# yannikkellerde/TD3

Hardware: AMD Instinct MI355X
Metric: TD3 gradient-steps/sec @ batch 256, HalfCheetah-v4, 1/2/4/8 GPU (higher is better)
Workload: dtype f32; 1 GPU; TD3_featured.train(replay_buffer, 256) on HalfCheetah-v4 shapes (state 17, action 6, actor 500-400-300, critic 2x 500-400-200, LayerNorm, policy_freq 2), replay 1e6 per GPU; global_batch=256, per_gpu_batch=256, replay_per_gpu=1000000, parallelism=single, launch=auto, norm=layer

## Files before the change

include/td3.h:

```cpp
#ifndef TD3_HIP_H
#define TD3_HIP_H

#include <stddef.h>
#include <stdint.h>

#ifdef __cplusplus
extern "C" {
#endif

typedef struct rb_handle rb_handle;
typedef struct td3_handle td3_handle;

typedef struct rb_info_t {
  int state_dim, action_dim;
  int record_floats;
  int64_t max_size, ptr, size;
  void* data;
  int device;
  int n_particles, particle_dim;
} rb_info_t;

int rb_create(int state_dim, int action_dim, int64_t max_size, int device, uint64_t seed,
              rb_handle** out);
int rb_destroy(rb_handle* h);
// ... 54 lines not shown
  double actor_loss;
  int actor_step;
  float* y;
  float* q1;
  float* q2;
  int64_t* idx;
  float* noise;
} td3_step_stats;

size_t td3_config_size(void);
int td3_default_config(td3_config* cfg, size_t cfg_size);
int td3_create(const td3_config* cfg, td3_handle** out);
int td3_destroy(td3_handle* h);

int td3_tensor_count(const td3_handle* h, int which_group );
int td3_tensor_info(const td3_handle* h, int which_group, int index, char* name, int name_len,
                    int64_t* rows, int64_t* cols);
int64_t td3_num_params(const td3_handle* h, int which_group);
int td3_get_params(td3_handle* h, int which, float* out, int64_t n);
int td3_set_params(td3_handle* h, int which, const float* in, int64_t n);
int td3_get_counters(const td3_handle* h, int64_t* total_it, int64_t* critic_step,
                     int64_t* actor_step);
int td3_set_counters(td3_handle* h, int64_t total_it, int64_t critic_step, int64_t actor_step);
int td3_set_adam(td3_handle* h, int group, double lr, double beta1, double beta2, double eps);
int td3_get_adam(const td3_handle* h, int group, double out[4] );

int td3_train_step(td3_handle* h, rb_handle* rb, int batch, void* stream,
                   const int64_t* inject_idx, const float* inject_noise, td3_step_stats* stats);
int td3_train_step_batch(td3_handle* h, const float* state, const float* action,
                         const float* next_state, const float* reward, const float* not_done,
                         int batch, void* stream, const float* inject_noise,
                         td3_step_stats* stats);
int td3_select_action(td3_handle* h, const float* state, float* action_out, int n);
int td3_eval_q(td3_handle* h, const float* state, const float* action, float* q_out, int n);

typedef struct td3_explore {
  float* x;
  float mu, theta, sigma;
  const uint8_t* reset;
  uint64_t seed, step;
  const float* inject_z;
  float* z_out;
} td3_explore;
int td3_select_action_device(td3_handle* h, const float* state, int n, const td3_explore* ex,
                             float* action_out, void* stream);
int td3_eval_q_device(td3_handle* h, const float* state, const float* action, int n, float* q_out, void* stream);

int td3_train_step_batch_particles(td3_handle* h, const float* feat, const float* part, const float* action,
                                   const float* next_feat, const float* next_part, const float* reward,
                                   const float* not_done, int batch, void* stream, const float* inject_noise,
                                   td3_step_stats* stats);
int td3_actor_learn_particles(td3_handle* h, const float* feat, const float* part, int batch, void* stream,
                              double* actor_loss);
int td3_select_action_particles(td3_handle* h, const float* feat, const float* part, float* action_out, int n);
int td3_eval_q_particles(td3_handle* h, const float* feat, const float* part, const float* action, float* q_out,
                         int n);
int td3_select_action_particles_device(td3_handle* h, const float* feat, const float* part, int n,
                                       const td3_explore* ex, float* action_out, void* stream);
int td3_eval_q_particles_device(td3_handle* h, const float* feat, const float* part, const float* action,
                                int n, float* q_out, void* stream);

int td3_comm_unique_id(unsigned char out[128]);
int td3_comm_init(td3_handle* h, const unsigned char id[128], int nranks, int rank);
int td3_dp_gather_optimizer_state(td3_handle* h);
int td3_comm_init_local(td3_handle** hs, int n);
int td3_train_step_local(td3_handle** hs, rb_handle** rbs, int n, int batch, const int64_t* inject_idx,
                         const float* inject_noise, td3_step_stats* stats);

int td3_sync(td3_handle* h);
void* td3_stream(td3_handle* h);
int td3_profile_stages(td3_handle* h, rb_handle* rb, int batch, int actor_phase, float* ms,
                       int max_stages, int* n_stages);
const char* td3_stage_name(td3_handle* h, int i);
const char* td3_stage_kernel(td3_handle* h, int i);
int td3_time_stage(td3_handle* h, int stage, int iters, float* ms_mean);
int td3_probe_kernel(td3_handle* h, rb_handle* rb, int batch, const char* kernel, int steps, float* ms_total,
                     int* launches);
double td3_stage_flops(td3_handle* h, int i);
double td3_stage_bytes(td3_handle* h, int i);
int td3_debug_activation(td3_handle* h, int eval, int layer, float* out, int rows, int cols);
int td3_debug_plan_flags(const td3_handle* h, int* flags);

int td3_debug_act_fail(td3_handle* h, int n);

const char* td3_last_error(void);

#ifdef __cplusplus
}
#endif
#endif
```

td3_amd/_lib.py:

```python
from __future__ import annotations

import atexit
import ctypes as C
import os

_HERE = os.path.dirname(os.path.abspath(__file__))
LIB_PATH = os.path.join(_HERE, "libtd3hip.so")


class rb_info_t(C.Structure):
    _fields_ = [("state_dim", C.c_int), ("action_dim", C.c_int), ("record_floats", C.c_int),
                ("max_size", C.c_int64), ("ptr", C.c_int64), ("size", C.c_int64),
                ("data", C.c_void_p), ("device", C.c_int),
                ("n_particles", C.c_int), ("particle_dim", C.c_int)]


class td3_config(C.Structure):
    _fields_ = [("struct_size", C.c_int), ("state_dim", C.c_int), ("action_dim", C.c_int),
                ("actor_hidden", C.c_int * 3), ("critic_hidden", C.c_int * 3),
                ("norm", C.c_int), ("max_action", C.c_float),
                ("discount", C.c_double), ("tau", C.c_double), ("policy_noise", C.c_double),
                ("noise_clip", C.c_double), ("policy_freq", C.c_int),
                ("lr", C.c_double), ("beta1", C.c_double), ("beta2", C.c_double),
                ("eps", C.c_double), ("seed", C.c_uint64), ("device", C.c_int),
# ... 1 lines not shown
                ("particle_dim", C.c_int), ("cdq", C.c_int)]


class td3_step_stats(C.Structure):
    _fields_ = [("critic_loss", C.c_double), ("actor_loss", C.c_double), ("actor_step", C.c_int),
                ("y", C.c_void_p), ("q1", C.c_void_p), ("q2", C.c_void_p), ("idx", C.c_void_p),
                ("noise", C.c_void_p)]


class td3_explore(C.Structure):
    _fields_ = [("x", C.c_void_p), ("mu", C.c_float), ("theta", C.c_float), ("sigma", C.c_float),
                ("reset", C.c_void_p), ("seed", C.c_uint64), ("step", C.c_uint64),
                ("inject_z", C.c_void_p), ("z_out", C.c_void_p)]


_P = C.c_void_p
_F = C.POINTER(C.c_float)
_D = C.POINTER(C.c_double)
_I64 = C.POINTER(C.c_int64)

SIGNATURES = {
    "rb_create": (C.c_int, [C.c_int, C.c_int, C.c_int64, C.c_int, C.c_uint64, C.POINTER(_P)]),
    "rb_destroy": (C.c_int, [_P]),
    "rb_info": (C.c_int, [_P, C.POINTER(rb_info_t)]),
    "rb_stream": (_P, [_P]),
    "rb_add": (C.c_int, [_P, _D, _D, _D, _D, _D, C.c_int64, _P]),
    "rb_add_records": (C.c_int, [_P, _F, C.c_int64, _P]),
    "rb_add_device": (C.c_int, [_P, _P, _P, _P, _P, _P, C.c_int64, _P]),
    "rb_add_particles_device": (C.c_int, [_P, _P, _P, _P, _P, _P, _P, _P, C.c_int64, _P]),
    "rb_fill_synthetic": (C.c_int, [_P, C.c_int64, C.c_float, C.c_uint64, _P]),
    "rb_sample": (C.c_int, [_P, C.c_int, _P, _P, _P, _P, _P, _P, _P, _P]),
    "rb_read_records": (C.c_int, [_P, C.c_int64, C.c_int64, _F]),
    "rb_write_records": (C.c_int, [_P, C.c_int64, C.c_int64, _F, C.c_int64, C.c_int64]),
    "rb_sync": (C.c_int, [_P]),
    "rb_create_particles": (C.c_int, [C.c_int, C.c_int, C.c_int, C.c_int, C.c_int64, C.c_int, C.c_uint64,
                                      C.POINTER(_P)]),
    "rb_add_particles": (C.c_int, [_P, _D, _D, _D, _D, _D, _D, _D, C.c_int64, _P]),
    "rb_sample_particles": (C.c_int, [_P, C.c_int, _P, _P, _P, _P, _P, _P, _P, _P, _P, _P]),
    "td3_config_size": (C.c_size_t, []),
    "td3_default_config": (C.c_int, [C.POINTER(td3_config), C.c_size_t]),
    "td3_create": (C.c_int, [C.POINTER(td3_config), C.POINTER(_P)]),
    "td3_destroy": (C.c_int, [_P]),
    "td3_tensor_count": (C.c_int, [_P, C.c_int]),
    "td3_tensor_info": (C.c_int, [_P, C.c_int, C.c_int, C.c_char_p, C.c_int, _I64, _I64]),
    "td3_num_params": (C.c_int64, [_P, C.c_int]),
    "td3_get_params": (C.c_int, [_P, C.c_int, _F, C.c_int64]),
    "td3_set_params": (C.c_int, [_P, C.c_int, _F, C.c_int64]),
    "td3_get_counters": (C.c_int, [_P, _I64, _I64, _I64]),
    "td3_set_counters": (C.c_int, [_P, C.c_int64, C.c_int64, C.c_int64]),
    "td3_set_adam": (C.c_int, [_P, C.c_int, C.c_double, C.c_double, C.c_double, C.c_double]),
    "td3_get_adam": (C.c_int, [_P, C.c_int, _D]),
    "td3_train_step": (C.c_int, [_P, _P, C.c_int, _P, _I64, _F, C.POINTER(td3_step_stats)]),
    "td3_train_step_batch": (C.c_int, [_P, _P, _P, _P, _P, _P, C.c_int, _P, _F,
                                       C.POINTER(td3_step_stats)]),
    "td3_select_action": (C.c_int, [_P, _F, _F, C.c_int]),
    "td3_eval_q": (C.c_int, [_P, _F, _F, _F, C.c_int]),
    "td3_select_action_device": (C.c_int, [_P, _P, C.c_int, C.POINTER(td3_explore), _P, _P]),
    "td3_eval_q_device": (C.c_int, [_P, _P, _P, C.c_int, _P, _P]),
    "td3_select_action_particles_device": (C.c_int, [_P, _P, _P, C.c_int, C.POINTER(td3_explore), _P, _P]),
    "td3_eval_q_particles_device": (C.c_int, [_P, _P, _P, _P, C.c_int, _P, _P]),
    "td3_train_step_batch_particles": (C.c_int, [_P, _P, _P, _P, _P, _P, _P, _P, C.c_int, _P, _F,
                                                 C.POINTER(td3_step_stats)]),
    "td3_actor_learn_particles": (C.c_int, [_P, _P, _P, C.c_int, _P, _D]),
    "td3_select_action_particles": (C.c_int, [_P, _F, _F, _F, C.c_int]),
    "td3_eval_q_particles": (C.c_int, [_P, _F, _F, _F, _F, C.c_int]),
    "td3_comm_unique_id": (C.c_int, [C.POINTER(C.c_ubyte)]),
    "td3_comm_init": (C.c_int, [_P, C.POINTER(C.c_ubyte), C.c_int, C.c_int]),
    "td3_comm_init_local": (C.c_int, [C.POINTER(_P), C.c_int]),
    "td3_dp_gather_optimizer_state": (C.c_int, [_P]),
    "td3_train_step_local": (C.c_int, [C.POINTER(_P), C.POINTER(_P), C.c_int, C.c_int, _I64, _F,
                                       C.POINTER(td3_step_stats)]),
    "td3_sync": (C.c_int, [_P]),
    "td3_stream": (_P, [_P]),
    "td3_profile_stages": (C.c_int, [_P, _P, C.c_int, C.c_int, _F, C.c_int, C.POINTER(C.c_int)]),
    "td3_stage_name": (C.c_char_p, [_P, C.c_int]),
    "td3_stage_kernel": (C.c_char_p, [_P, C.c_int]),
    "td3_time_stage": (C.c_int, [_P, C.c_int, C.c_int, _F]),
    "td3_probe_kernel": (C.c_int, [_P, _P, C.c_int, C.c_char_p, C.c_int, _F, C.POINTER(C.c_int)]),
    "td3_stage_flops": (C.c_double, [_P, C.c_int]),
    "td3_stage_bytes": (C.c_double, [_P, C.c_int]),
    "td3_debug_activation": (C.c_int, [_P, C.c_int, C.c_int, _P, C.c_int, C.c_int]),
    "td3_debug_plan_flags": (C.c_int, [_P, _P]),
    "td3_debug_act_fail": (C.c_int, [_P, C.c_int]),
    "td3_last_error": (C.c_char_p, []),
}

TD3_ACTOR, TD3_ACTOR_TARGET, TD3_CRITIC, TD3_CRITIC_TARGET = 0, 1, 2, 3
TD3_ACTOR_ADAM_M, TD3_ACTOR_ADAM_V, TD3_CRITIC_ADAM_M, TD3_CRITIC_ADAM_V = 4, 5, 6, 7
TD3_ACTOR_GRAD, TD3_CRITIC_GRAD = 8, 9

_lib = None
_shutting_down = False


def _mark_shutdown():
    global _shutting_down
    _shutting_down = True


atexit.register(_mark_shutdown)


def alive() -> bool:
    return _lib is not None and not _shutting_down


def load(path: str = LIB_PATH):
    global _lib
    if _lib is not None:
        return _lib
    import torch
    path = os.environ.get("TD3_LIB", path)
    if not os.path.exists(path):
        raise ImportError(
            f"libtd3hip.so not found at {path}: build it with `python -m td3_amd.build` "
            "(hipcc --offload-arch=gfx950). There is no CPU fallback.")
    lib = C.CDLL(path, mode=C.RTLD_GLOBAL)
    for name, (res, args) in SIGNATURES.items():
        fn = getattr(lib, name)
        fn.restype = res
        fn.argtypes = args
    _lib = lib
    return lib


class TD3Error(RuntimeError):
    pass


def check(rc: int, what: str = ""):
    if rc != 0:
        msg = _lib.td3_last_error().decode(errors="replace") if _lib is not None else ""
        raise TD3Error(f"{what} failed ({rc}): {msg}")


def default_config():
    lib = load()
    if C.sizeof(td3_config) != lib.td3_config_size():
        raise TD3Error(f"td3_config binding is {C.sizeof(td3_config)} bytes, libtd3hip's "
                       f"{lib.td3_config_size()}: td3_amd/_lib.py is out of date with include/td3.h")
    cfg = td3_config()
    check(lib.td3_default_config(C.byref(cfg), C.sizeof(cfg)), "td3_default_config")
    return cfg


def fptr(a):
    return a.ctypes.data_as(_F)


def i64ptr(a):
    return a.ctypes.data_as(_I64)


def dptr(a):
    return a.ctypes.data_as(_D)
```

td3_amd/csrc/common.h:

```cpp
#pragma once
#include <hip/hip_runtime.h>
#include <stdint.h>
#include <stddef.h>

#define TD3_EV_FLAGS (hipEventDisableTiming | hipEventReleaseToDevice)

namespace td3 {
void set_error(const char* fmt, ...);
}

#define TD3_HIP(expr)                                                              \
  do {                                                                             \
    hipError_t _e = (expr);                                                        \
    if (_e != hipSuccess) {                                                        \
      td3::set_error("%s:%d %s -> %s", __FILE__, __LINE__, #expr,                  \
                     hipGetErrorString(_e));                                       \
      return -2;                                                                   \
    }                                                                              \
  } while (0)

#define TD3_ARG(cond, msg)                                                         \
  do {                                                                             \
    if (!(cond)) {                                                                 \
      td3::set_error("argument error: %s (%s)", msg, #cond);                        \
// ... 1 lines not shown
    }                                                                              \
  } while (0)

#define TD3_RC(expr)          \
  do {                        \
    int _rc = (expr);         \
    if (_rc) return _rc;      \
  } while (0)

namespace td3 {

constexpr int kWave = 64;
constexpr int kTile = 32;

__host__ __device__ inline int pad32(int x) { return (x + 31) & ~31; }
__host__ __device__ inline int pad4(int x) { return (x + 3) & ~3; }

__host__ __device__ inline int lds_stride(int kp) { return kp + ((4 - kp) % 64 + 64) % 64; }

struct u32x4 { uint32_t x, y, z, w; };

__device__ __forceinline__ u32x4 philox4x32_10(u32x4 ctr, uint32_t k0, uint32_t k1) {
  const uint32_t M0 = 0xD2511F53u, M1 = 0xCD9E8D57u;
  const uint32_t W0 = 0x9E3779B9u, W1 = 0xBB67AE85u;
#pragma unroll
  for (int i = 0; i < 10; ++i) {
    uint32_t hi0 = __umulhi(M0, ctr.x), lo0 = M0 * ctr.x;
    uint32_t hi1 = __umulhi(M1, ctr.z), lo1 = M1 * ctr.z;
    ctr = u32x4{hi1 ^ ctr.y ^ k0, lo1, hi0 ^ ctr.w ^ k1, lo0};
    k0 += W0;
    k1 += W1;
  }
  return ctr;
}

enum : uint32_t { kStreamIndex = 1u, kStreamNoise = 2u, kStreamFill = 3u, kStreamExplore = 4u };

__device__ __forceinline__ uint64_t philox_index(uint64_t seed, uint64_t step, uint32_t row,
                                                 uint64_t n) {
  u32x4 c{row, kStreamIndex, (uint32_t)step, (uint32_t)(step >> 32)};
  u32x4 r = philox4x32_10(c, (uint32_t)seed, (uint32_t)(seed >> 32));
  uint64_t bits = ((uint64_t)r.x << 32) | r.y;
  return __umul64hi(bits, n);
}

__device__ __forceinline__ float u01_open(uint32_t x) {
  return ((float)(x >> 8) + 1.0f) * (1.0f / 16777216.0f);
}

__device__ __forceinline__ void philox_normal4(uint64_t seed, uint64_t step, uint32_t stream,
                                               uint32_t idx, float out[4]) {
  u32x4 c{idx, stream, (uint32_t)step, (uint32_t)(step >> 32)};
  u32x4 r = philox4x32_10(c, (uint32_t)seed, (uint32_t)(seed >> 32));
  float u1 = u01_open(r.x), u2 = u01_open(r.y), u3 = u01_open(r.z), u4 = u01_open(r.w);
  constexpr float kM2Ln2 = -2.0f * 0.693147180559945f;
  const float rad1 = __builtin_amdgcn_sqrtf(kM2Ln2 * __builtin_amdgcn_logf(u1));
  const float rad2 = __builtin_amdgcn_sqrtf(kM2Ln2 * __builtin_amdgcn_logf(u3));
  const float s1 = __builtin_amdgcn_sinf(u2), c1 = __builtin_amdgcn_cosf(u2);
  const float s2 = __builtin_amdgcn_sinf(u4), c2 = __builtin_amdgcn_cosf(u4);
  out[0] = rad1 * c1;
  out[1] = rad1 * s1;
  out[2] = rad2 * c2;
  out[3] = rad2 * s2;
}

__device__ __forceinline__ float wave_sum(float v) {
#pragma unroll
  for (int o = 32; o > 0; o >>= 1) v += __shfl_xor(v, o, 64);
  return v;
}

typedef float f32x16 __attribute__((ext_vector_type(16)));

__device__ __forceinline__ f32x16 mfma32x32x2(float a, float b, f32x16 c) {
  return __builtin_amdgcn_mfma_f32_32x32x2f32(a, b, c, 0, 0, 0);
}

__device__ __forceinline__ int mfma_row(int r, int lane) { return (r & 3) + 8 * (r >> 2) + 4 * (lane >> 5); }

struct Counters {
  int64_t total_it;
  int64_t critic_step;
  int64_t actor_step;
  int64_t pad;
  double pw[4];
  double beta[4];
};

}
```

td3_amd/csrc/kernels.h:

```cpp
#pragma once
#include "common.h"

#ifndef TD3_GEMM_WAVES
#define TD3_GEMM_WAVES 8
#endif

namespace td3 {

constexpr int kGemmWaves = TD3_GEMM_WAVES;

enum Pro : int {
  kProCopy = 0,
  kProLN = 1,
  kProLNBwd = 2,
  kProGather = 3,
  kProL0 = 4,
  kProL0G = 5,
  kProHeadBwd = 6,
};
constexpr int kL0XS = 36;

enum RowKind : int {
  kRowPolicyHead = 0,
  kRowActorHeadBwd = 3,
// ... 355 lines not shown
  int gen_noise;
};

constexpr int kGemvRows = 4;
struct GemvProb {
  const float* X; int ldx; int K;
  const float* lng; const float* lnb;
  const float* W; int ldw; const float* b; int N;
  float* Y; int ldy;
};
struct GemvArgs {
  GemvProb p[2];
  int B;
};
int launch_gemv(const GemvArgs& a, int nprob, hipStream_t s);

constexpr int kGemv0K = 64;
constexpr int kGemvQ = kGemvRows * kGemv0K + 4;
struct Gemv01Args {
  GemvArgs l1;
  const float* W0[2]; const float* b0[2];
  int ldw0, K0, N0;
  float xq[kGemvQ];
};
int launch_gemv01(const Gemv01Args& a, int nprob, hipStream_t s);

struct ActArgs {
  Gemv01Args g;
  GemvProb l2[2];
  HeadProb head[2];
  int* ctr;
  float max_action;
  unsigned* flag;
  unsigned seq;
  int fail_test;
};
constexpr unsigned kActFailed = 0x80000000u;
constexpr int kActFailInc = 1 << 16;
int launch_act(const ActArgs& a, int nprob, hipStream_t s);

struct LnBwdProb {
  const float* GU; const float* H; const float* stats; const float* lng; int ld, K;
  float* GZ;
};
constexpr int kMaxLnBwd = 3;
struct LnBwdTable {
  LnBwdProb p[kMaxLnBwd];
};

struct DwProb {
  const float* G; int ldg;
  const float* U; int ldu;
  int Np, Kp;
  int64_t offW, offb;
  int64_t offg, offbeta;
  const float* GU; int ldgu;
  const float* H; int ldh; const float* stats;
  int ntk;
  int tile_begin;
  const float* rs; int ldrs;
  int kvalid;
};

enum DwMode : int { kDwGrad = 0, kDwAdam = 1, kDwAdamPolyak = 2 };

struct AdamArgs {
  float* P; float* G; float* M; float* V; float* T;
  float* P4; float* T4;
  const Counters* ctr; int which;
  double lr, beta1, beta2, eps;
  float tau;
  float grad_scale;
};

constexpr int kMaxDwProbs = 10;
struct DwArgs {
  DwProb probs[kMaxDwProbs]; int nprob; int Bp;
  AdamArgs adam;
  int mode;
  int tile64;
  int scaled;
};

struct DwTile {
  int prob;
  int kind;
  int a, b;
};
struct DwSplit {
  const DwTile* tiles; int ntile;
  int S;
  int G;
  int J;
  int tm;
  int slot;
  const int* wg_unit;
  const int* tile_wg;
  float* slab;
};
int launch_dw_split(const DwArgs& a, const DwSplit& k, hipStream_t s);

constexpr int kBumpActorOnly = 2;
int launch_gemm(int mode, int wn, int pro, const GemmTable& t, int nblocks, int Bp, int lds_bytes,
                Counters* bump, int bump_actor, hipStream_t s);
int launch_l0r16(int nct, int wk, int gather, const GemmTable& t, int nblocks, int Bp, Counters* bump,
                 int bump_actor, hipStream_t s);
int l0r16_lds_bytes(int Kp, int nct, int wk);
int gemm2_supported(int m1, int w1, int p1, int m2, int w2, int p2);
int launch_gemm2(int m1, int w1, int p1, const GemmTable& t1, int nb1, int m2, int w2, int p2, const GemmTable& t2,
                 int nb2, int Bp, int lds, hipStream_t s);
int launch_rows(int kind, const GemmTable& t, int Bp, hipStream_t s);
int launch_rows2(int kind1, int kind2, int n1, const GemmTable& t, int Bp, hipStream_t s);
int launch_heads(const HeadArgs& a, int nprob, hipStream_t s);
int launch_lnbwd_rows(const LnBwdTable& tab, int nprob, int Bp, int norm, hipStream_t s);
int launch_dw(const DwArgs& a, int nblocks, hipStream_t s);
struct W4Map {
  float* P4; float* T4;
  int64_t base;
  int nmat;
  int64_t off[8]; int Np[8], Kp[8];
};
int launch_adam_flat(const AdamArgs& a, int64_t n, int polyak, hipStream_t s, const W4Map* w4 = nullptr);
int launch_polyak_w4(float* T, const float* P, int64_t n, float tau, const W4Map& w, hipStream_t s);
constexpr int kMaxLocalReplicas = 8;
struct LocalSumArgs {
  float* a[kMaxLocalReplicas];
  int n;
  int64_t size;
};
int launch_local_sum(const LocalSumArgs& a, hipStream_t s);

struct WnLinear {
  int64_t offW, offb, offg, offv;
  int N, K, ld;
  int row0;
};
constexpr int kMaxWnLinears = 8;
struct WnArgs {
  WnLinear lin[kMaxWnLinears];
  int nlin, rows;
  AdamArgs adam;
  int mode;
  int polyak;
  float* arena; float* arena2;
};
enum WnMode : int { kWnDerive = 0, kWnAdam = 1 };
int launch_wn(const WnArgs& a, hipStream_t s);
int launch_polyak_flat(float* T, const float* P, int64_t n, float tau, hipStream_t s);
constexpr int kMaxW4Mats = 16;
struct W4PackArgs {
  const float* src[2]; float* dst[2]; int npair;
  int64_t off[kMaxW4Mats]; int Np[kMaxW4Mats], Kp[kMaxW4Mats]; int64_t first[kMaxW4Mats + 1];
  int nmat;
};
int launch_w4_pack(const W4PackArgs& a, hipStream_t s);
struct ExploreArgs {
  const float* pi; int ldp;
  float* action_out;
  int n, ad;
  int plain;
  float max_action;
  float* x;
  float mu, theta, sigma;
  const uint8_t* reset;
  uint64_t seed, step;
  const float* inject_z;
// ... 7 lines not shown
```

td3_amd/csrc/kernels.hip:

```cpp
#include <math.h>
#include <stdlib.h>

#include "dev.h"
#include "kernels.h"

namespace td3 {

#ifdef TD3_TL
__device__ unsigned long long td3_tl[8192][8];
__device__ unsigned long long td3_clk[8192][2];
__device__ __forceinline__ void tl_mark(int k) {
  const unsigned id = blockIdx.x + blockIdx.y * gridDim.x;
  if (threadIdx.x == 0 && id < 8192) {
    if (k == 3) asm volatile("s_waitcnt vmcnt(0)" ::: "memory");
    if (k == 1 || k == 2) td3_clk[id][k - 1] = __builtin_amdgcn_s_memtime();
    td3_tl[id][k] = __builtin_amdgcn_s_memrealtime();
    if (k == 0) {
      unsigned x, hw;
      asm volatile("s_getreg_b32 %0, hwreg(HW_REG_XCC_ID)" : "=s"(x));
      asm volatile("s_getreg_b32 %0, hwreg(HW_REG_HW_ID)" : "=s"(hw));
      td3_tl[id][4] = x | ((unsigned long long)hw << 32);
    }
  }
}
// ... 796 lines not shown
  rv_load(gu[0], P.ex[kDUin] + (size_t)c.row * ldin, ldin, c.lane);
  rv_load(xr[0], P.ex[kXin] + (size_t)c.row * ldin, ldin, c.lane);
  rv_load(h3[0], P.ex[kH3] + (size_t)c.row * ld3, ld3, c.lane);
  if (NORM) {
    rv_load(gi, P.ex[kGammaIn], ldin, c.lane);
    rv_load(g3, P.ex[kGamma3], ld3, c.lane);
    mi[0] = gld(P.ex[kStatsIn] + c.row);
    ri[0] = gld(P.ex[kStatsIn] + (c.Bp + c.row));
    mn3[0] = gld(P.ex[kStats3] + c.row);
    rs3[0] = gld(P.ex[kStats3] + (c.Bp + c.row));
  } else {
    mi[0] = mn3[0] = 0.f;
    ri[0] = rs3[0] = 1.f;
  }
  const float tl = c.lane < ad ? gld(P.ex[kTanh] + ((size_t)c.row * 32 + c.lane)) : 0.f;
  ln_bwd_rows<1, false>(gu, xr, gi, mi, ri, Kin, c.lane, NORM);
  const bool live = c.row < P.B;
  float gu3[1][8];
#pragma unroll
  for (int jj = 0; jj < 8; ++jj) gu3[0][jj] = 0.f;
  for (int o = 0; o < ad; ++o) {
    const int col = acol + o;
    const int jsel = ((col >> 8) << 2) + (col & 3);
    float v = 0.f;
#pragma unroll
    for (int jj = 0; jj < 8; ++jj) v = jj == jsel ? gu[0][jj] : v;
    const float ga = __shfl(v, (col & 255) >> 2, 64);
    const float t = __shfl(tl, o, 64);
    const float gz4 = live ? (ga * ma) * (1.f - t * t) : 0.f;
    if (c.lane == 0) gst(P.ex[kDZ4] + ((size_t)c.row * 32 + o), gz4);
    float w4[8];
    rv_load(w4, P.ex[kW4] + (size_t)o * ldw4, ld3, c.lane);
#pragma unroll
    for (int jj = 0; jj < 8; ++jj) gu3[0][jj] += gz4 * w4[jj];
  }
  rv_store(P.ex[kDU3] + (size_t)c.row * ld3, ld3, c.lane, gu3[0]);
  ln_bwd_rows<1>(gu3, h3, g3, mn3, rs3, K3, c.lane, NORM);
  rv_store(P.Aout + (size_t)c.row * P.ldao, P.ldao, c.lane, gu3[0]);
}

#ifndef TD3_ROW_WAVES
#define TD3_ROW_WAVES 1
#endif
constexpr int kRowWaves = TD3_ROW_WAVES;
template <bool NORM>
__device__ __forceinline__ void row_unit_loss(const GemmProb& P, const RowCtx& c) {
  using namespace unit_loss;
  asm volatile("" ::"s"(P.ex[kH3]), "s"(P.ex[kGamma3]), "s"(P.ex[kBeta3]), "s"(P.ex[kW4]), "s"(P.ex[kB4]),
               "s"(P.ex[kQ]), "s"(P.ex[kU3]), "s"(P.ex[kStats3]), "s"(P.ex[kDU3]), "s"(P.exi[kK3]), "s"(P.exi[kLd3]),
               "s"(P.Aout), "s"(P.ldao));
  const int K3 = P.exi[kK3], ld3 = P.exi[kLd3];
  float x[1][8], h[1][8], g[8], bb[8], w[8], mean[1] = {0.f}, rstd[1] = {1.f};
  rv_load(x[0], P.ex[kH3] + (size_t)c.row * ld3, ld3, c.lane);
  if (NORM) {
    rv_load(g, P.ex[kGamma3], ld3, c.lane);
    rv_load(bb, P.ex[kBeta3], ld3, c.lane);
  } else {
#pragma unroll
    for (int jj = 0; jj < 8; ++jj) g[jj] = bb[jj] = 0.f;
  }
  rv_load(w, P.ex[kW4], ld3, c.lane);
  const float b4 = gld(P.ex[kB4]);
  __builtin_amdgcn_sched_barrier(0);
#pragma unroll
  for (int jj = 0; jj < 8; ++jj) h[0][jj] = x[0][jj];
  if (NORM) ln_fwd_rows<1>(x, g, bb, K3, c.lane, mean, rstd);
  const float q = wsum(rv_pdot(x[0], w, K3, c.lane)) + b4;
  if (c.lane == 0) {
    gst(P.ex[kQ] + c.row, q);
    if (NORM) {
      gst(P.ex[kStats3] + c.row, mean[0]);
      gst(P.ex[kStats3] + (c.Bp + c.row), rstd[0]);
    }
  }
  if (NORM) rv_store(P.ex[kU3] + (size_t)c.row * ld3, ld3, c.lane, x[0]);
  float gu[1][8];
#pragma unroll
  for (int jj = 0; jj < 8; ++jj) gu[0][jj] = w[jj];
  rv_store(P.ex[kDU3] + (size_t)c.row * ld3, ld3, c.lane, gu[0]);
  ln_bwd_rows<1>(gu, h, g, mean, rstd, K3, c.lane, NORM);
  rv_store(P.Aout + (size_t)c.row * P.ldao, P.ldao, c.lane, gu[0]);
}

template <bool NORM>
__device__ __forceinline__ void row_target_loss(const GemmProb& P, const RowCtx& c) {
  using namespace target_loss;
  asm volatile("" ::"s"(P.ex[kH3]), "s"(P.ex[kH3 + 1]), "s"(P.ex[kGamma3]), "s"(P.ex[kGamma3 + 1]), "s"(P.ex[kBeta3]),
               "s"(P.ex[kBeta3 + 1]), "s"(P.ex[kW4]), "s"(P.ex[kW4 + 1]), "s"(P.ex[kB4]), "s"(P.ex[kB4 + 1]),
               "s"(P.ex[kReward]), "s"(P.ex[kNotDone]), "s"(P.ex[kQ]), "s"(P.ex[kQ + 1]), "s"(P.exi[kK3]),
               "s"(P.exi[kLd3]));
  asm volatile("" ::"s"(P.ex[kY]), "s"(P.ex[kDZ4]), "s"(P.ex[kDZ4 + 1]), "s"(P.ex[kSqErr]), "s"(P.ex[kG]),
               "s"(P.ex[kG + 1]), "s"(P.exf[kDiscount]), "s"(P.exf[kGradScale]), "s"(P.B));
  const int K3 = P.exi[kK3], ld3 = P.exi[kLd3];
  float x0[1][8], x1[1][8], g[2][8], bb[2][8], w[2][8];
  rv_load(x0[0], P.ex[kH3] + (size_t)c.row * ld3, ld3, c.lane);
  rv_load(x1[0], P.ex[kH3 + 1] + (size_t)c.row * ld3, ld3, c.lane);
#pragma unroll
  for (int n = 0; n < 2; ++n) {
    if (NORM) {
      rv_load(g[n], P.ex[kGamma3 + n], ld3, c.lane);
      rv_load(bb[n], P.ex[kBeta3 + n], ld3, c.lane);
    }
    rv_load(w[n], P.ex[kW4 + n], ld3, c.lane);
  }
  const float b40 = gld(P.ex[kB4]), b41 = gld(P.ex[kB4 + 1]);
  const float rw = gld(P.ex[kReward] + c.row), nd = gld(P.ex[kNotDone] + c.row);
  const float q1 = gld(P.ex[kQ] + c.row), q2 = gld(P.ex[kQ + 1] + c.row);
  __builtin_amdgcn_sched_barrier(0);
  float m0[1], s0[1], m1[1], s1[1];
  if (NORM) {
    ln_fwd_rows<1>(x0, g[0], bb[0], K3, c.lane, m0, s0);
    ln_fwd_rows<1>(x1, g[1], bb[1], K3, c.lane, m1, s1);
  }
  const float d0 = rv_pdot(x0[0], w[0], K3, c.lane);
  const float d1 = rv_pdot(x1[0], w[1], K3, c.lane);
  const float tq0 = wsum(d0) + b40, tq1 = wsum(d1) + b41;
  const float y = rw + (nd * P.exf[kDiscount]) * fminf(tq0, tq1);
  const bool live = c.row < P.B;
  const float e1 = q1 - y, e2 = q2 - y;
  const float g1 = live ? P.exf[kGradScale] * e1 : 0.f, g2 = live ? P.exf[kGradScale] * e2 : 0.f;
  if (c.lane == 0) {
    gst(P.ex[kY] + c.row, y);
    gst(P.ex[kDZ4] + ((size_t)c.row * 32), g1);
    gst(P.ex[kDZ4 + 1] + ((size_t)c.row * 32), g2);
    gst(P.ex[kSqErr] + c.row, live ? e1 * e1 : 0.f);
    gst(P.ex[kSqErr] + (c.Bp + c.row), live ? e2 * e2 : 0.f);
    gst(P.ex[kG] + c.row, g1);
    gst(P.ex[kG + 1] + c.row, g2);
  }
}

template <bool NORM>
__device__ __forceinline__ void row_lnbwd(const GemmProb& P, const RowCtx& c) {
  using namespace ln_bwd;
  asm volatile("" ::"s"(P.ex[kDU]), "s"(P.ex[kH]), "s"(P.ex[kStats]), "s"(P.ex[kGamma]), "s"(P.ex[kDZ]),
               "s"(P.exi[kLd]), "s"(P.exi[kK]));
  const int ld = P.exi[kLd];
  float gu[1][8], h[1][8], g[8], mean[1], rstd[1];
  float4 qg[2], qu[2], qh[2];
  if constexpr (NORM) rv_load_raw(qg, P.ex[kGamma], ld, c.lane);
  rv_load_raw(qu, P.ex[kDU] + (size_t)c.row * ld, ld, c.lane);
  rv_load_raw(qh, P.ex[kH] + (size_t)c.row * ld, ld, c.lane);
  mean[0] = NORM ? gld(P.ex[kStats] + c.row) : 0.f;
  rstd[0] = NORM ? gld(P.ex[kStats] + (c.Bp + c.row)) : 1.f;
  __builtin_amdgcn_sched_barrier(0);
  if constexpr (NORM) rv_from_raw(g, qg, ld, c.lane);
  else {
#pragma unroll
    for (int jj = 0; jj < 8; ++jj) g[jj] = 0.f;
  }
  rv_from_raw(gu[0], qu, ld, c.lane);
  rv_from_raw(h[0], qh, ld, c.lane);
  if constexpr (NORM) ln_bwd_rows_pk<1>(gu, h, g, mean, rstd, 1.0f / (float)P.exi[kK]);
  else ln_bwd_rows<1>(gu, h, g, mean, rstd, P.exi[kK], c.lane, 0);
  rv_store(P.ex[kDZ] + (size_t)c.row * ld, ld, c.lane, gu[0]);
}

template <int KIND, bool NORM, int RW>
__device__ __forceinline__ void row_dispatch(const GemmProb& P, const RowCtx& c) {
  if constexpr (KIND == kRowPolicyHead) row_policy_head<NORM, RW>(P, c);
  else if constexpr (KIND == kRowActorHeadBwd) row_actor_head_bwd<NORM, RW>(P, c);
  else if constexpr (KIND == kRowCriticLossP) row_critic_loss_p<NORM>(P, c);
  else if constexpr (KIND == kRowActorLossP) row_actor_loss_p<NORM>(P, c);
  else if constexpr (KIND == kRowActorHeadBwdP) row_actor_head_bwd_p<NORM>(P, c);
  else if constexpr (KIND == kRowUnitLoss) row_unit_loss<NORM>(P, c);
  else if constexpr (KIND == kRowTargetLoss) row_target_loss<NORM>(P, c);
  else if constexpr (KIND == kRowLnBwd) row_lnbwd<NORM>(P, c);
}

template <int KIND, bool NORM, int RW = kRowWaves>
__global__ __launch_bounds__(64 * RW) void row_kernel(int Bp, GemmTable tab) {
  const GemmProb& P = tab.p[blockIdx.y];
  const RowCtx c{(int)(blockIdx.x * RW + (threadIdx.x >> 6)), (int)(threadIdx.x & 63), Bp};
  TL_MARK(0);
  row_dispatch<KIND, NORM, RW>(P, c);
  TL_MARK(3);
}

template <int K1, int K2, bool NORM, int RW = kRowWaves>
__global__ __launch_bounds__(64 * RW) void row_kernel2(int Bp, int n1, GemmTable tab) {
  const GemmProb& P = tab.p[blockIdx.y];
  const RowCtx c{(int)(blockIdx.x * RW + (threadIdx.x >> 6)), (int)(threadIdx.x & 63), Bp};
  TL_MARK(0);
  if ((int)blockIdx.y < n1) row_dispatch<K1, NORM, RW>(P, c);
  else row_dispatch<K2, NORM, RW>(P, c);
  TL_MARK(3);
}


__device__ __forceinline__ int w_sk(int wsk) { return wsk ? wsk : 4; }
__device__ __forceinline__ int w0_sn(int w0sk) { return w0sk ? 4 : 32; }
__device__ __forceinline__ int w0_sk(int w0sk) { return w0sk ? w0sk : 4; }

template <int MODE>
__device__ __forceinline__ void load_chunk(const GemmProb& P, float (&b)[16], int ch, int ncol, int h) {
  const int kb = ch * 32 + 16 * h;
  if (MODE == 0) {
    const int sk = w_sk(P.wsk);
    const float* wp = P.W + (size_t)ncol * P.ldw + (size_t)(kb >> 2) * sk;
#pragma unroll
    for (int q = 0; q < 4; ++q) {
      const float4 v = gld4(wp + (size_t)q * sk);
      b[4 * q + 0] = v.x; b[4 * q + 1] = v.y; b[4 * q + 2] = v.z; b[4 * q + 3] = v.w;
    }
  } else {
    const float* wp = P.W + (size_t)kb * P.ldw + ncol;
#pragma unroll
    for (int s = 0; s < 16; ++s) b[s] = gld(wp + (size_t)s * P.ldw);
  }
}

// ... 1004 lines not shown
    if (ok[e]) any = idx[e];
  if (any < 0) return;
#pragma unroll
  for (int e = 0; e < N; ++e) {
    const int64_t j = ok[e] ? idx[e] : any;
    st.mm[e] = gld(a.adam.M + j);
    st.vv[e] = gld(a.adam.V + j);
    st.pp[e] = gld(a.adam.P + j);
    st.tt[e] = pol ? gld(a.adam.T + j) : 0.f;
  }
}

template <int N>
__device__ __forceinline__ void apply_grads_loaded(const DwArgs& a, const AdamK& k, const int64_t (&idx)[N],
                                                   const float (&g)[N], const bool (&ok)[N], AdamState<N>& st,
                                                   const int64_t* qidx = nullptr) {
  if (a.mode == kDwGrad) {
#pragma unroll
    for (int e = 0; e < N; ++e)
      if (ok[e]) gst(a.adam.G + idx[e], g[e]);
    return;
  }
  const bool pol = a.mode == kDwAdamPolyak;
  float (&mm)[N] = st.mm;
  float (&vv)[N] = st.vv;
  float (&pp)[N] = st.pp;
  float (&tt)[N] = st.tt;
#pragma unroll
  for (int e = 0; e < N; ++e) {
    mm[e] = __fmaf_rn(k.w1, g[e] - mm[e], mm[e]);
    vv[e] = vv[e] * k.b2;
    vv[e] = vv[e] + (k.c2 * g[e]) * g[e];
    const float denom = sqrtf(vv[e]) / k.bc2s + k.eps;
    pp[e] = pp[e] + (k.negss * mm[e]) / denom;
    tt[e] = k.tau * pp[e] + k.omt * tt[e];
  }
#pragma unroll
  for (int e = 0; e < N; ++e) {
    if (!ok[e]) continue;
    sst(a.adam.M + idx[e], mm[e]);
    sst(a.adam.V + idx[e], vv[e]);
    pst(a.adam.P + idx[e], pp[e]);
    if (pol) pst(a.adam.T + idx[e], tt[e]);
    if (qidx && a.adam.P4) {
      pst(a.adam.P4 + qidx[e], pp[e]);
      if (pol) pst(a.adam.T4 + qidx[e], tt[e]);
    }
  }
}

template <int N>
__device__ __forceinline__ void apply_grads(const DwArgs& a, const AdamK& k, const int64_t (&idx)[N],
                                            const float (&g)[N], const bool (&ok)[N], const int64_t* qidx = nullptr) {
  AdamState<N> st;
  adam_state_load<N>(a, idx, ok, st);
  apply_grads_loaded<N>(a, k, idx, g, ok, st, qidx);
}

template <bool SC>
__device__ __forceinline__ void dw_load_chunk(const DwProb& P, int rc, int h, int n0, int k0, int i,
                                              float (&av)[16], float (&bv)[16], float4 (&sc)[4]) {
  const int rb = rc * 32 + 16 * h;
  const float* gp = P.G + (size_t)rb * P.ldg + n0 + i;
  const float* up = P.U + (size_t)rb * P.ldu + k0 + i;
#pragma unroll
  for (int s = 0; s < 16; ++s) {
    av[s] = gld(gp + (size_t)s * P.ldg);
    bv[s] = gld(up + (size_t)s * P.ldu);
  }
  if constexpr (SC) {
#pragma unroll
    for (int q = 0; q < 4; ++q) sc[q] = gld4(P.rs + (size_t)(rb + 4 * q) * P.ldrs);
  }
}
template <bool SC>
__device__ __forceinline__ void dw_scale(float (&av)[16], const float4 (&sc)[4]) {
  if constexpr (!SC) return;
#pragma unroll
  for (int q = 0; q < 4; ++q) {
    av[4 * q + 0] *= sc[q].x; av[4 * q + 1] *= sc[q].y; av[4 * q + 2] *= sc[q].z; av[4 * q + 3] *= sc[q].w;
  }
}

template <int NT, bool SC>
__device__ __forceinline__ void dw_vector_tile_cols(const DwArgs& a, const DwProb& P, const AdamK& k, int j,
                                               float* red) {
  constexpr int NG = NT / 32;
  const int n0 = j * 32;
  const int c = threadIdx.x & 31, rg = threadIdx.x >> 5;
  const bool ln = P.offg >= 0;
  const bool hasb = P.offb >= 0;
  float sb = 0.f, sg = 0.f, sbeta = 0.f;
  for (int r0 = rg; r0 < a.Bp; r0 += 8 * NG) {
    float gz[8], gu[8], hh[8], mu[8], rs[8];
#pragma unroll
    for (int u = 0; u < 8; ++u) {
      const int r = min(r0 + NG * u, a.Bp - 1);
      const float sc = SC ? gld(P.rs + (size_t)r * P.ldrs) : 1.f;
      gz[u] = hasb ? gld(P.G + ((size_t)r * P.ldg + n0 + c)) * sc : 0.f;
      if (ln) {
        gu[u] = gld(P.GU + ((size_t)r * P.ldgu + n0 + c)) * sc;
        hh[u] = gld(P.H + ((size_t)r * P.ldh + n0 + c));
        mu[u] = gld(P.stats + r);
        rs[u] = gld(P.stats + (a.Bp + r));
      }
      if (r0 + NG * u >= a.Bp) {
        gz[u] = 0.f;
        gu[u] = 0.f;
      }
    }
#pragma unroll
    for (int u = 0; u < 8; ++u) {
      sb += gz[u];
      if (ln) {
        sg += gu[u] * ((hh[u] - mu[u]) * rs[u]);
        sbeta += gu[u];
      }
    }
  }
  red[(0 * NG + rg) * 32 + c] = sb;
  red[(1 * NG + rg) * 32 + c] = sg;
  red[(2 * NG + rg) * 32 + c] = sbeta;
  __syncthreads();
  if (threadIdx.x < 32) {
    float s0 = 0.f, s1 = 0.f, s2 = 0.f;
#pragma unroll
    for (int g = 0; g < NG; ++g) {
      s0 += red[(0 * NG + g) * 32 + c];
      s1 += red[(1 * NG + g) * 32 + c];
      s2 += red[(2 * NG + g) * 32 + c];
    }
    const int64_t idx[3] = {P.offb + n0 + c, P.offg + n0 + c, P.offbeta + n0 + c};
    const float gq[3] = {s0, s1, s2};
    const bool ok[3] = {hasb, ln, ln};
    apply_grads<3>(a, k, idx, gq, ok);
  }
}

template <int NT, bool SC, int U = 8>
__device__ __forceinline__ void dw_vector_tile(const DwArgs& a, const DwProb& P, const AdamPw& pw, int j,
                                               float* red) {
  constexpr int RG = NT / 8;
  const int n0 = j * 32;
  const int c4 = (threadIdx.x & 7) * 4, rg = threadIdx.x >> 3;
  const bool ln = P.offg >= 0;
  const bool hasb = P.offb >= 0;
  const int c = threadIdx.x & 31;
  const int64_t idx[3] = {P.offb + n0 + c, P.offg + n0 + c, P.offbeta + n0 + c};
  const bool ok[3] = {hasb, ln, ln};
  AdamState<3> st;
  float sb[4] = {0.f, 0.f, 0.f, 0.f}, sg[4] = {0.f, 0.f, 0.f, 0.f}, sbeta[4] = {0.f, 0.f, 0.f, 0.f};
  const float* gzp = hasb ? P.G : P.GU;
  const float* gup = ln ? P.GU : P.G;
  const float* hp = ln ? P.H : P.G;
  const float* stp = ln ? P.stats : P.G;
  const int ldz = hasb ? P.ldg : P.ldgu, ldu = ln ? P.ldgu : P.ldg, ldh = ln ? P.ldh : P.ldg;
  for (int r0 = rg; r0 < a.Bp; r0 += RG * U) {
    float4 gz[U], gu[U], hh[U];
    float mu[U], rs[U], sc[U];
#pragma unroll
    for (int u = 0; u < U; ++u) {
      const int r = min(r0 + RG * u, a.Bp - 1);
      gz[u] = gld4(gzp + ((size_t)r * ldz + n0 + c4));
      gu[u] = gld4(gup + ((size_t)r * ldu + n0 + c4));
      hh[u] = gld4(hp + ((size_t)r * ldh + n0 + c4));
      mu[u] = gld(stp + r);
      rs[u] = gld(stp + (a.Bp + r));
      sc[u] = SC ? gld(P.rs + (size_t)r * P.ldrs) : 1.f;
    }
    if (r0 == rg && threadIdx.x < 32) adam_state_load<3>(a, idx, ok, st);
    __builtin_amdgcn_sched_barrier(0);
    if (!hasb) {
#pragma unroll
      for (int u = 0; u < U; ++u) gz[u] = make_float4(0.f, 0.f, 0.f, 0.f);
    }
#pragma unroll
    for (int u = 0; u < U; ++u) {
      if (r0 + RG * u >= a.Bp) continue;
      const float z[4] = {gz[u].x * sc[u], gz[u].y * sc[u], gz[u].z * sc[u], gz[u].w * sc[u]};
      sb[0] += z[0]; sb[1] += z[1]; sb[2] += z[2]; sb[3] += z[3];
      if (ln) {
        const float g4[4] = {gu[u].x * sc[u], gu[u].y * sc[u], gu[u].z * sc[u], gu[u].w * sc[u]};
        const float h4[4] = {hh[u].x, hh[u].y, hh[u].z, hh[u].w};
#pragma unroll
        for (int e = 0; e < 4; ++e) {
          sg[e] += g4[e] * ((h4[e] - mu[u]) * rs[u]);
          sbeta[e] += g4[e];
        }
      }
    }
  }
#pragma unroll
  for (int e = 0; e < 4; ++e) {
    red[(0 * RG + rg) * 33 + c4 + e] = sb[e];
    red[(1 * RG + rg) * 33 + c4 + e] = sg[e];
    red[(2 * RG + rg) * 33 + c4 + e] = sbeta[e];
  }
  __syncthreads();
  TL_MARK(1);
  TL_MARK(2);
  if (threadIdx.x < 32) {
    float s0 = 0.f, s1 = 0.f, s2 = 0.f;
#pragma unroll 8
    for (int g = 0; g < RG; ++g) {
      s0 += red[(0 * RG + g) * 33 + c];
      s1 += red[(1 * RG + g) * 33 + c];
      s2 += red[(2 * RG + g) * 33 + c];
    }
    const float gq[3] = {s0, s1, s2};
    apply_grads_loaded<3>(a, make_adam(a.adam, pw), idx, gq, ok, st);
  }
  TL_MARK(3);
}

#ifndef TD3_DW_OCC
#define TD3_DW_OCC 3
#endif
template <bool SC>
__global__ __launch_bounds__(256, TD3_DW_OCC) void dw_kernel(DwArgs a, int nb) {
  __shared__ float red[4 * 32 * 33];
  const int b = xcd_tile(nb);
  TL_MARK(0);
  if (b >= nb) return;
  int pi = 0;
#pragma unroll
  for (int i = 1; i < kMaxDwProbs; ++i)
    if (i < a.nprob && b >= a.probs[i].tile_begin) pi = i;
  const DwProb& P = a.probs[pi];
  const int t = b - P.tile_begin;
  const int nmat = (P.Np >> 5) * P.ntk;
  const AdamPw pw = adam_pw(a.adam);
  if (t < nmat) {
    const int kt = t % P.ntk, nt = t / P.ntk;
    const int n0 = nt * 32, k0 = kt * 32;
    const int wave = threadIdx.x >> 6, lane = threadIdx.x & 63;
    const int i = lane & 31, h = lane >> 5;
    const int nrc = a.Bp >> 5;
    const int cb = wave * nrc / 4, ce = (wave + 1) * nrc / 4;
    f32x16 acc;
#pragma unroll
    for (int r = 0; r < 16; ++r) acc[r] = 0.f;
    float a0[16], b0[16], a1[16], b1[16];
    float4 c0[4], c1[4];
    if (cb < ce) dw_load_chunk<SC>(P, cb, h, n0, k0, i, a0, b0, c0);
    if (cb + 1 < ce) dw_load_chunk<SC>(P, cb + 1, h, n0, k0, i, a1, b1, c1);
    const int tn = threadIdx.x >> 3, tq = (threadIdx.x & 7) * 4;
    const int64_t ix = P.offW + (int64_t)(n0 + tn) * P.Kp + k0 + tq;
    const bool grad_only = a.mode == kDwGrad, pol = a.mode == kDwAdamPolyak;
    float4 sm4 = make_float4(0.f, 0.f, 0.f, 0.f), sv4 = sm4, sp4 = sm4, st4 = sm4;
    if (!grad_only) {
      sm4 = gld4(a.adam.M + ix);
      sv4 = gld4(a.adam.V + ix);
      sp4 = gld4(a.adam.P + ix);
      st4 = gld4((pol ? a.adam.T : a.adam.P) + ix);
    }
    for (int rc = cb; rc < ce; rc += 2) {
      dw_scale<SC>(a0, c0);
#pragma unroll
      for (int s = 0; s < 16; ++s) acc = mfma32x32x2(a0[s], b0[s], acc);
      if (rc + 2 < ce) dw_load_chunk<SC>(P, rc + 2, h, n0, k0, i, a0, b0, c0);
      if (rc + 1 >= ce) break;
      dw_scale<SC>(a1, c1);
#pragma unroll
      for (int s = 0; s < 16; ++s) acc = mfma32x32x2(a1[s], b1[s], acc);
      if (rc + 3 < ce) dw_load_chunk<SC>(P, rc + 3, h, n0, k0, i, a1, b1, c1);
    }
    TL_MARK(5);
#pragma unroll
    for (int r = 0; r < 16; ++r) red[(wave * 32 + mfma_row(r, lane)) * 33 + i] = acc[r];
    __syncthreads();
    TL_MARK(1);
    TL_MARK(2);
    const AdamK k = make_adam(a.adam, pw);
    float gq[4];
#pragma unroll
    for (int q = 0; q < 4; ++q) {
      float g = red[tn * 33 + tq + q];
#pragma unroll
      for (int w = 1; w < 4; ++w) g = g + red[(w * 32 + tn) * 33 + tq + q];
      gq[q] = k0 + tq + q < P.kvalid ? g : 0.f;
    }
    if (grad_only) {
      gst4(a.adam.G + ix, make_float4(gq[0], gq[1], gq[2], gq[3]));
    } else {
      float mm[4] = {sm4.x, sm4.y, sm4.z, sm4.w}, vv[4] = {sv4.x, sv4.y, sv4.z, sv4.w};
      float pp[4] = {sp4.x, sp4.y, sp4.z, sp4.w}, tt[4] = {st4.x, st4.y, st4.z, st4.w};
#pragma unroll
      for (int e = 0; e < 4; ++e) {
        mm[e] = __fmaf_rn(k.w1, gq[e] - mm[e], mm[e]);
        vv[e] = vv[e] * k.b2;
        vv[e] = vv[e] + (k.c2 * gq[e]) * gq[e];
        const float denom = sqrtf(vv[e]) / k.bc2s + k.eps;
        pp[e] = pp[e] + (k.negss * mm[e]) / denom;
        tt[e] = k.tau * pp[e] + k.omt * tt[e];
      }
      sst4(a.adam.M + ix, make_float4(mm[0], mm[1], mm[2], mm[3]));
      sst4(a.adam.V + ix, make_float4(vv[0], vv[1], vv[2], vv[3]));
      pst4(a.adam.P + ix, make_float4(pp[0], pp[1], pp[2], pp[3]));
      if (pol) pst4(a.adam.T + ix, make_float4(tt[0], tt[1], tt[2], tt[3]));
      if (a.adam.P4) {
        const int64_t iq = P.offW + ((int64_t)((k0 + tq) >> 2) * P.Np + n0 + tn) * 4;
        pst4(a.adam.P4 + iq, make_float4(pp[0], pp[1], pp[2], pp[3]));
        if (pol) pst4(a.adam.T4 + iq, make_float4(tt[0], tt[1], tt[2], tt[3]));
      }
    }
    TL_MARK(3);
    return;
  }
  dw_vector_tile<256, SC>(a, P, pw, t - nmat, red);
}

constexpr int kDw64S = 66;
constexpr int kDw64Depth = 2;
#ifndef TD3_DW64_VEC4
#define TD3_DW64_VEC4 1
#endif
template <bool SC>
__global__ __launch_bounds__(512) void dw64_kernel(DwArgs a, int nb) {
  __shared__ float sm[2 * 2 * 64 * kDw64S];
  __shared__ float4 ssl4[2][16];
  const int b = xcd_tile(nb);
  TL_MARK(0);
  if (b >= nb) return;
  int pi = 0;
#pragma unroll
  for (int i = 1; i < kMaxDwProbs; ++i)
    if (i < a.nprob && b >= a.probs[i].tile_begin) pi = i;
  const DwProb& P = a.probs[pi];
  const int t = b - P.tile_begin;
  const int ntn = (P.Np + 63) >> 6;
  const int nmat = ntn * P.ntk;
  const AdamPw pw = adam_pw(a.adam);
  if (t >= nmat) {
#if TD3_DW64_VEC4
    dw_vector_tile<512, SC, 4>(a, P, pw, t - nmat, sm);
#else
    dw_vector_tile_cols<512, SC>(a, P, make_adam(a.adam, pw), t - nmat, sm);
#endif
#ifdef TD3_TL
    if (threadIdx.x == 0 && blockIdx.x < 8192) td3_tl[blockIdx.x][6] = 1;
#endif
    TL_MARK(3);
    return;
  }
  const int kt = t % P.ntk, nt = t / P.ntk;
  const int n0 = nt * 64, k0 = kt * 64;
  const int tid = threadIdx.x, wave = tid >> 6, lane = tid & 63, i = lane & 31, h = lane >> 5;
  const int qn = (wave >> 1) & 1, qk = wave & 1, rh = wave >> 2;
  constexpr int D = kDw64Depth;
  float4 sg[D][2], su[D][2];
  float ssc[D];
  auto fetch = [&](int r0, float4 (&g)[2], float4 (&u)[2], float& sc) {
#pragma unroll
    for (int v = 0; v < 2; ++v) {
      const int e = tid + 512 * v, row = r0 + (e >> 4), c4 = (e & 15) * 4;
      const bool live = row < a.Bp;
      g[v] = (live && n0 + c4 < P.Np) ? gld4(P.G + (size_t)row * P.ldg + n0 + c4) : make_float4(0.f, 0.f, 0.f, 0.f);
      u[v] = (live && k0 + c4 < P.Kp) ? gld4(P.U + (size_t)row * P.ldu + k0 + c4) : make_float4(0.f, 0.f, 0.f, 0.f);
    }
    if constexpr (SC) sc = gld(P.rs + (size_t)min(r0 + (tid & 63), a.Bp - 1) * P.ldrs);
  };
  auto put = [&](int buf, const float4 (&gq)[2], const float4 (&uq)[2], float sc) {
    float* g = sm + buf * 2 * 64 * kDw64S;
    float* uu = g + 64 * kDw64S;
#pragma unroll
    for (int v = 0; v < 2; ++v) {
      const int e = tid + 512 * v, row = e >> 4, c4 = (e & 15) * 4;
      float* gp = g + row * kDw64S + c4;
      float* up = uu + row * kDw64S + c4;
      gp[0] = gq[v].x; gp[1] = gq[v].y; gp[2] = gq[v].z; gp[3] = gq[v].w;
      up[0] = uq[v].x; up[1] = uq[v].y; up[2] = uq[v].z; up[3] = uq[v].w;
    }
    if constexpr (SC) {
      if (tid < 64) reinterpret_cast<float*>(ssl4[buf])[tid] = sc;
    }
  };
  f32x16 acc;
#pragma unroll
  for (int r = 0; r < 16; ++r) acc[r] = 0.f;
  const int nstep = (a.Bp + 63) >> 6;
#pragma unroll
  for (int d = 0; d < D; ++d)
    if (d < nstep) fetch(d * 64, sg[d], su[d], ssc[d]);
  for (int st0 = 0; st0 < nstep; st0 += D) {
#pragma unroll
    for (int d = 0; d < D; ++d) {
      const int st = st0 + d;
      if (st >= nstep) break;
      const int buf = st & 1;
      put(buf, sg[d], su[d], ssc[d]);
      __syncthreads();
      if (st + D < nstep) fetch((st + D) * 64, sg[d], su[d], ssc[d]);
// ... 921 lines not shown
    ok = p1.K == a.g.N0 && p1.N >= 1 && p1.N <= 512 && p2.K == p1.N && p2.X == p1.Y && p2.N >= 1 && p2.N <= p1.N &&
         hd.H3 == p2.Y && hd.K3 == p2.N && hd.nout >= 1 && hd.nout <= 64 && hd.ldw <= 512;
  }
  if (!ok) {
    set_error("launch_act: unsupported query shape (%d problems, %d rows, layer 0 %d -> %d)", nprob, B, a.g.K0, a.g.N0);
    return -1;
  }
  for (int k = 1; k < nprob; ++k)
    if (a.g.l1.p[k].N != N1) {
      set_error("launch_act: networks of one launch need the same layer-1 width");
      return -1;
    }
  const dim3 grid((N1 + 15) / 16, nprob);
  if (a.g.ldw0 < (a.g.K0 <= 32 ? 32 : 64)) {
    set_error("launch_act: layer-0 rows of %d floats (K0 %d)", a.g.ldw0, a.g.K0);
    return -1;
  }
  if (a.g.K0 <= 32) {
    if (B == 1) hipLaunchKernelGGL((act_kernel<1, 8>), grid, dim3(256), 0, s, a);
    else if (B == 2) hipLaunchKernelGGL((act_kernel<2, 8>), grid, dim3(256), 0, s, a);
    else hipLaunchKernelGGL((act_kernel<4, 8>), grid, dim3(256), 0, s, a);
  } else {
    if (B == 1) hipLaunchKernelGGL((act_kernel<1, 16>), grid, dim3(256), 0, s, a);
    else if (B == 2) hipLaunchKernelGGL((act_kernel<2, 16>), grid, dim3(256), 0, s, a);
    else hipLaunchKernelGGL((act_kernel<4, 16>), grid, dim3(256), 0, s, a);
  }
  TD3_HIP(hipGetLastError());
  return 0;
}

int launch_gemv01(const Gemv01Args& a, int nprob, hipStream_t s) {
  int N = 0;
  for (int k = 0; k < nprob; ++k) N = std::max(N, a.l1.p[k].N);
  if (nprob < 1 || nprob > 2 || a.l1.B < 1 || a.l1.B > kGemvRows || a.K0 < 1 || a.K0 > kGemv0K ||
      a.N0 > 512 || a.N0 < 1) {
    set_error("launch_gemv01: %d problems, %d rows, layer 0 %d -> %d (max 2, %d, %d -> 512)", nprob, a.l1.B, a.K0,
              a.N0, kGemvRows, kGemv0K);
    return -1;
  }
  for (int k = 0; k < nprob; ++k)
    if (a.l1.p[k].K != a.N0 || a.l1.p[k].K > 512) {
      set_error("launch_gemv01: layer-1 input width %d != layer-0 width %d", a.l1.p[k].K, a.N0);
      return -1;
    }
  const dim3 grid((N + 15) / 16, nprob);
  if (a.l1.B == 1) hipLaunchKernelGGL(gemv01_kernel<1>, grid, dim3(256), 0, s, a);
  else if (a.l1.B == 2) hipLaunchKernelGGL(gemv01_kernel<2>, grid, dim3(256), 0, s, a);
  else hipLaunchKernelGGL(gemv01_kernel<4>, grid, dim3(256), 0, s, a);
  TD3_HIP(hipGetLastError());
  return 0;
}

int launch_lnbwd_rows(const LnBwdTable& tab, int nprob, int Bp, int norm, hipStream_t s) {
  if (nprob < 1 || nprob > kMaxLnBwd || Bp % (kRowWaves * kLnBwdRB) != 0) {
    set_error("launch_lnbwd_rows: %d problems (max %d), Bp %d (multiple of %d)", nprob, kMaxLnBwd, Bp, kRowWaves * kLnBwdRB);
    return -1;
  }
  if (norm) hipLaunchKernelGGL(lnbwd_rows_kernel<true>, dim3(Bp / (kRowWaves * kLnBwdRB), nprob), dim3(64 * kRowWaves), 0, s, Bp, tab);
  else hipLaunchKernelGGL(lnbwd_rows_kernel<false>, dim3(Bp / (kRowWaves * kLnBwdRB), nprob), dim3(64 * kRowWaves), 0, s, Bp, tab);
  TD3_HIP(hipGetLastError());
  return 0;
}

#ifndef TD3_DW64G
#define TD3_DW64G 1
#endif
int launch_dw(const DwArgs& a, int nblocks, hipStream_t s) {
  if (nblocks <= 0) return 0;
  const dim3 grid((nblocks + 7) & ~7);
  if (a.tile64 && (a.Bp & 63) == 0 && TD3_DW64G) {
    if (a.scaled) hipLaunchKernelGGL(dw64g_kernel<true>, grid, dim3(512), 0, s, a, nblocks);
    else hipLaunchKernelGGL(dw64g_kernel<false>, grid, dim3(512), 0, s, a, nblocks);
  } else if (a.tile64) {
    if (a.scaled) hipLaunchKernelGGL(dw64_kernel<true>, grid, dim3(512), 0, s, a, nblocks);
    else hipLaunchKernelGGL(dw64_kernel<false>, grid, dim3(512), 0, s, a, nblocks);
  } else {
    if (a.scaled) hipLaunchKernelGGL(dw_kernel<true>, grid, dim3(256), 0, s, a, nblocks);
    else hipLaunchKernelGGL(dw_kernel<false>, grid, dim3(256), 0, s, a, nblocks);
  }
  TD3_HIP(hipGetLastError());
  return 0;
}

int launch_dw_split(const DwArgs& a, const DwSplit& k, hipStream_t s) {
  if (k.ntile <= 0) return 0;
  if (k.G <= 0 || (k.G & 7) || k.S <= 0 || (a.Bp & 63) || a.Bp != 64 * k.S || (k.tm != 64 && k.tm != 128) ||
      k.slot < k.tm * k.tm || k.J <= 0) {
    set_error("launch_dw_split: bad split (G %d, S %d, tm %d, slot %d, J %d, Bp %d)", k.G, k.S, k.tm, k.slot,
              k.J, a.Bp);
    return -1;
  }
  if (k.tm == 128) {
    if (a.scaled) hipLaunchKernelGGL((dwsk_kernel<true, true>), dim3(k.G), dim3(512), 0, s, a, k);
    else hipLaunchKernelGGL((dwsk_kernel<false, true>), dim3(k.G), dim3(512), 0, s, a, k);
  } else {
    if (a.scaled) hipLaunchKernelGGL((dwsk_kernel<true, false>), dim3(k.G), dim3(512), 0, s, a, k);
    else hipLaunchKernelGGL((dwsk_kernel<false, false>), dim3(k.G), dim3(512), 0, s, a, k);
  }
  hipLaunchKernelGGL(dwsk_combine_kernel, dim3(4 * k.ntile), dim3(256), 0, s, a, k);
  TD3_HIP(hipGetLastError());
  return 0;
}

int launch_adam_flat(const AdamArgs& a, int64_t n, int polyak, hipStream_t s, const W4Map* w4) {
  auto al16 = [](const float* p) { return ((uintptr_t)p & 15) == 0; };
  if ((n & 3) || !al16(a.P) || !al16(a.G) || !al16(a.M) || !al16(a.V) || (polyak && !al16(a.T))) {
    set_error("launch_adam_flat: the range must be float4-aligned (n %% 4 == 0, 16-B aligned arenas)");
    return -1;
  }
  W4Map w{};
  if (w4 && w4->P4) {
    w = *w4;
    bool ok = w.nmat >= 1 && w.nmat <= 8 && (w.base & 3) == 0 && (!polyak || w.T4);
    for (int m = 0; ok && m < w.nmat; ++m) ok = (w.off[m] & 3) == 0 && w.Kp[m] % 4 == 0;
    if (!ok) {
      set_error("launch_adam_flat: bad k-quad image map");
      return -1;
    }
  }
  const int blocks = (int)std::min<int64_t>((n / 4 + 255) / 256, 2048);
  hipLaunchKernelGGL(adam_flat_kernel, dim3(blocks), dim3(256), 0, s, a, n, polyak, w);
  TD3_HIP(hipGetLastError());
  return 0;
}

int launch_wn(const WnArgs& a, hipStream_t s) {
  if (a.nlin < 1 || a.nlin > kMaxWnLinears || a.rows < 1) {
    set_error("launch_wn: %d linears (max %d), %d rows", a.nlin, kMaxWnLinears, a.rows);
    return -1;
  }
  for (int l = 0; l < a.nlin; ++l)
    if (a.lin[l].K < 1 || a.lin[l].K > 512) {
      set_error("launch_wn: input width %d (max 512)", a.lin[l].K);
      return -1;
    }
  hipLaunchKernelGGL(wn_kernel, dim3((a.rows + 3) / 4), dim3(256), 0, s, a);
  TD3_HIP(hipGetLastError());
  return 0;
}

int launch_local_sum(const LocalSumArgs& a, hipStream_t s) {
  if (a.n < 1 || a.n > kMaxLocalReplicas || a.size < 0) {
    set_error("launch_local_sum: %d replicas (max %d)", a.n, kMaxLocalReplicas);
    return -1;
  }
  const int blocks = (int)std::min<int64_t>((a.size + 255) / 256, 2048);
  if (blocks > 0) hipLaunchKernelGGL(local_sum_kernel, dim3(blocks), dim3(256), 0, s, a);
  TD3_HIP(hipGetLastError());
  return 0;
}

__global__ __launch_bounds__(256) void w4_pack_kernel(W4PackArgs a) {
  const int64_t total = a.first[a.nmat];
  for (int64_t e = blockIdx.x * 256 + threadIdx.x; e < (int64_t)a.npair * total; e += (int64_t)gridDim.x * 256) {
    const int pr = (int)(e / total);
    const int64_t q = e - (int64_t)pr * total;
    int m = 0;
    while (m + 1 < a.nmat && q >= a.first[m + 1]) ++m;
    const int64_t pc = q - a.first[m];
    const int kq = a.Kp[m] >> 2;
    const int n = (int)(pc / kq), j = (int)(pc - (int64_t)n * kq);
    const float4 v = gld4(a.src[pr] + a.off[m] + (int64_t)n * a.Kp[m] + 4 * j);
    gst4(a.dst[pr] + a.off[m] + ((int64_t)j * a.Np[m] + n) * 4, v);
  }
}

// ... 170 lines not shown
```

td3_amd/csrc/td3.hip:

```cpp
#include <rccl/rccl.h>
#include <stdarg.h>
#include <stdio.h>
#include <string.h>

#include <algorithm>
#include <atomic>
#include <chrono>
#include <cmath>
#include <cstdlib>
#include <functional>
#include <map>
#include <memory>
#include <string>
#include <vector>

#include "encoder.h"
#include "kernels.h"
#include "replay.h"
#include "../../include/td3.h"

namespace td3 {

static thread_local char g_err[1024] = "";

// ... 83 lines not shown
  for (int l = 0; l < 3; ++l) {
    LNormL& Ln = n.ln[l];
    Ln.N = dims[l + 1];
    Ln.Np = pad32(Ln.N);
    Ln.offg = off;
    off += Ln.Np;
    Ln.offb = off;
    off += Ln.Np;
    if (norm) {
      tensors.push_back({prefix + "lnorms." + std::to_string(l) + ".weight", Ln.N, 0, Ln.offg, 0});
      tensors.push_back({prefix + "lnorms." + std::to_string(l) + ".bias", Ln.N, 0, Ln.offb, 0});
    }
  }
  return n;
}

struct EvalB {
  float* X = nullptr; int ldx = 0;
  float* H[3] = {};
  float* U[3] = {};
  float* stats[3] = {};
  float* GU[3] = {};
  float* GZ[4] = {};
  float* T = nullptr;
  float* Qv = nullptr;
  float* Uin = nullptr;
  float* statsIn = nullptr;
  float* GUin = nullptr;
  uint64_t* mask = nullptr;
  float* partial = nullptr;
  float* gpool = nullptr;
};

struct Scratch {
  float* base = nullptr;
  size_t cap = 0, used = 0;
  float* take(size_t floats) {
    size_t n = (floats + 63) & ~(size_t)63;
    float* p = base + used;
    used += n;
    return p;
  }
};

struct GemmLaunch {
  int mode, wn, pro;
  GemmTable t;
  int blocks, Bp, lds;
  bool plain;
};

struct Stage {
  std::string name;
  std::function<int(hipStream_t)> run;
  double flops = 0;
  std::string kernel;
  double bytes = 0;
  std::shared_ptr<GemmLaunch> gemm;
  int collective = -1;
  int64_t coll_off = 0, coll_n = -1;
  std::function<int(hipStream_t)> after;
  int64_t coll_slice = 0;
};

struct LocalGroup {
  std::vector<td3_handle*> hs;
};

struct SlabRef {
  float* p = nullptr;
  size_t bytes = 0;
};

struct Plan {
  int B = 0, Bp = 0;
  SlabRef dwslab;
  bool dp_overlap = false;
  float* scratch = nullptr;
  size_t scratch_bytes = 0;
  float *X_SA = nullptr, *X_S2A = nullptr, *X_SP = nullptr;
  int ld_sa = 0;
  float *R = nullptr, *ND = nullptr, *noise = nullptr, *Y = nullptr, *sqerr = nullptr;
  float* gscale[2] = {};
  float* W1aT = nullptr;
  int64_t* d_idx = nullptr;
  int64_t* d_inject_idx = nullptr;
  EvalB TA, Q[2], A, TQ[2], AQ;
  std::vector<void*> tables;
  std::vector<Stage> body[2][2];
  std::vector<Stage> body_ring[2][2];
  RingSide rside{};
  bool fuse_gather = false;
  bool w4 = false;
  hipGraphExec_t graph[2][2] = {{nullptr, nullptr}, {nullptr, nullptr}};
  hipGraphExec_t graph_g[2][2] = {{nullptr, nullptr}, {nullptr, nullptr}};
  uint64_t graph_ring_gen = 0;
  int particles = 0;
  int nq = 1, ldq = 1;
  int ld_a = 0, ld_q = 0;
  float *XA = nullptr, *XTA = nullptr, *XAQ = nullptr, *XQ[2] = {}, *XTQ[2] = {};
  float* pbatch = nullptr;
  int64_t* d_iota = nullptr;
  const float* src_data = nullptr;
  int src_rec = 0, src_op = 0, src_op2 = 0;
  const int64_t* src_idx = nullptr;
  uint64_t src_key = 0;
  int nwg = 0;
  int nwg_a = 0;
  std::vector<Stage> actor_learn;
};

constexpr int kMappedRows = 256;

struct ActPlan {
  int Bp = 0;
  float* scratch = nullptr;
  float* hio = nullptr;
  float *X_S = nullptr, *X_SA = nullptr, *out = nullptr, *q[2] = {nullptr, nullptr};
  float *XQ2 = nullptr, *pbatch = nullptr;
  float *hX_S = nullptr, *hX_SA = nullptr, *hout = nullptr, *hq[2] = {nullptr, nullptr};
  float *hXQ2 = nullptr, *hpbatch = nullptr;
  int ldo = 0;
  bool gemv = false, gemv01 = false;
  GemvArgs gv_act[3], gv_q[3];
  Gemv01Args g01_act{}, g01_q{};
  HeadArgs head_act{}, head_q{};
  bool act1 = false;
  ActArgs a1_act{}, a1_q{};
  unsigned* hflag[2] = {nullptr, nullptr};
  unsigned seq[2] = {0, 0};
  int fail_test = 0;
  int64_t* d_iota = nullptr;
  const float* dev_part = nullptr;
  int dev_n = 0;
  EvalB A, Q[2];
  std::vector<void*> tables;
  std::vector<Stage> act, evalq;
};

struct IoCarve {
  Scratch* S;
  float* h = nullptr;
  float* d = nullptr;
  size_t used = 0;
  float* take(size_t floats, float** host) {
    if (!h) {
      *host = nullptr;
      return S->take(floats);
    }
    const size_t n = (floats + 63) & ~(size_t)63;
    *host = h + used;
    float* p = d + used;
    used += n;
    return p;
  }
};

static int map_io(ActPlan* A, size_t floats, IoCarve* io) {
  if (A->Bp > kMappedRows) return 0;
  TD3_HIP(hipHostMalloc(&A->hio, floats * 4, hipHostMallocMapped));
  memset(A->hio, 0, floats * 4);
  void* d = nullptr;
  TD3_HIP(hipHostGetDevicePointer(&d, A->hio, 0));
  io->h = A->hio;
  io->d = static_cast<float*>(d);
  return 0;
}

}

using namespace td3;

struct td3_handle {
  td3_config cfg;
  int sd, ad;
  int particles = 0, N = 0, D = 0, cdq = 1;
  Group actor, critic;
  float* arena = nullptr;
  Counters* d_ctr = nullptr;
  float* ones = nullptr;
  int64_t total_it = 0, critic_step = 0, actor_step = 0;
  struct AdamHp { double lr, beta1, beta2, eps; } adam[2];
  hipStream_t stream = nullptr;
  hipStream_t act_stream = nullptr;
  hipStream_t actor_stream = nullptr;
  hipEvent_t actor_ev = nullptr;
  bool actor_ev_pending = false;
  bool act_used = false;
  hipStream_t last_step_stream = nullptr;
  std::unique_ptr<Plan> plan;
  std::map<int, std::unique_ptr<ActPlan>> act;
  std::map<int, std::unique_ptr<ActPlan>> act_dev;
  hipStream_t dev_stream = nullptr;
  hipEvent_t dev_ev = nullptr;
  ncclComm_t comm = nullptr;
  hipStream_t comm_stream = nullptr;
  hipEvent_t comm_ev = nullptr, comm_ev1 = nullptr, comm_done = nullptr;
  std::shared_ptr<LocalGroup> local;
  int nranks = 1, rank = 0;
  bool dp_sharded = false;
  bool w4_build = false;
  int64_t opt_gathered_it = -1;
  std::vector<Stage>* last_body = nullptr;
  Ring* last_ring = nullptr;
  uint64_t last_ring_gen = 0;
  bool probing = false;
  std::string probe_kernel;
  std::vector<hipEvent_t> probe_ev;
  int probe_used = 0;
  std::vector<std::string> stage_names;
  std::vector<std::string> stage_kernels;
};

namespace td3 {

static int upload(td3_handle* h, std::vector<void*>& owned, const void* host, size_t bytes, void** out) {
  void* d = nullptr;
  TD3_HIP(hipMalloc(&d, bytes));
  TD3_HIP(hipMemcpy(d, host, bytes, hipMemcpyHostToDevice));
  owned.push_back(d);
  *out = d;
  (void)h;
  return 0;
}

static void alloc_eval(Scratch& S, const NetL& n, int Bp, float* X, int ldx, bool bwd, bool norm,
                       bool policy_or_q, EvalB& e) {
  e.X = X;
  e.ldx = ldx;
  for (int l = 0; l < 3; ++l) {
    const int Np = n.lin[l].Np;
    e.H[l] = S.take((size_t)Bp * Np);
    e.U[l] = norm ? S.take((size_t)Bp * Np) : e.H[l];
    e.stats[l] = S.take((size_t)2 * Bp);
    if (bwd) {
      e.GU[l] = S.take((size_t)Bp * Np);
      e.GZ[l] = S.take((size_t)Bp * Np);
    }
  }
  if (bwd) e.GZ[3] = S.take((size_t)Bp * 32);
  if (policy_or_q) {
    e.T = S.take((size_t)Bp * 32);
    e.Qv = S.take((size_t)Bp * 32);
  }
  if (n.D > 0) {
    const int Kp0 = n.lin[0].Kp;
    e.Uin = norm ? S.take((size_t)Bp * Kp0) : X;
    e.statsIn = S.take((size_t)2 * Bp);
    if (bwd) e.GUin = S.take((size_t)Bp * Kp0);
  }
}

static int gemm_lds_bytes(int Kp, int rt = 1) {
  int f = std::max(32 * rt * lds_stride(Kp), kGemmWaves * 32 * 33);
  return f * 4;
}

struct RingOut {
  float* a; int lda;
  float* b; int ldb;
  float* r; float* nd;
};

// ... 547 lines not shown
#define TD3_DWSK 1
#endif
#ifndef TD3_DWSK_G
#define TD3_DWSK_G 256
#endif
constexpr int kDwSplitWorkgroups = TD3_DWSK_G;
static int dwsk_tile_edge() { return env_int("TD3_DWSK_T", 64) == 128 ? 128 : 64; }
static int dwsk_matrix_weight() { return std::max(1, env_int("TD3_DWSK_WM", 6)); }

static bool dp_overlap(const td3_handle* h) {
  const int m = env_int("TD3_DP_BUCKETS", 0);
  if (m <= 0) return false;
  if (h->local) return true;
  return h->comm && (h->nranks > 1 || m >= 2);
}

static bool dp_shard(const td3_handle* h) {
  const int m = env_int("TD3_DP_SHARD", 0);
  return m == 2 || (m == 1 && h->nranks > 1);
}
static int64_t shard_slice(const Group& g, int nranks) { return ((g.size + 4 * nranks - 1) / (4 * nranks)) * 4; }

static int make_dw_split(td3_handle* h, std::vector<void*>& owned, const DwArgs& a, SlabRef* slab, DwSplit& out) {
  const int tm = dwsk_tile_edge();
  const int wm = dwsk_matrix_weight();
  std::vector<DwTile> tiles;
  std::vector<int> wt;
  for (int pi = 0; pi < a.nprob; ++pi) {
    const DwProb& p = a.probs[pi];
    if (p.ntk > 0) {
      for (int nt = 0; nt < (p.Np + tm - 1) / tm; ++nt)
        for (int kt = 0; kt < (p.Kp + tm - 1) / tm; ++kt) {
          tiles.push_back(DwTile{pi, 0, nt, kt});
          const int an = std::min(tm, p.Np - nt * tm) / 32, ak = std::min(tm, p.Kp - kt * tm) / 32;
          const int q = tm == 128 ? (an > 2 ? 2 : 1) * (ak > 2 ? 2 : 1) : 1;
          wt.push_back(2 + wm * q / 4);
        }
    }
    for (int j = 0; j < p.Np / 32; ++j) {
      tiles.push_back(DwTile{pi, 1, j, 0});
      wt.push_back(1);
    }
  }
  DwSplit k{};
  k.ntile = (int)tiles.size();
  k.S = a.Bp / 64;
  k.G = kDwSplitWorkgroups;
  k.tm = tm;
  k.slot = tm * tm;
  const int units = k.ntile * k.S;
  int64_t wtot = 0;
  for (int w : wt) wtot += (int64_t)w * k.S;
  const int64_t cw = (wtot + k.G - 1) / k.G;
  std::vector<int> idx(k.G + 1 + 2 * k.ntile, units);
  std::vector<int> vu(units);
  int64_t pos = 0;
  int vcur = 0;
  idx[0] = 0;
  for (int u = 0; u < units; ++u) {
    const int w = wt[u / k.S];
    const int v = (int)std::min<int64_t>(k.G - 1, (2 * pos + w) / (2 * cw));
    while (vcur < v) idx[++vcur] = u;
    vu[u] = v;
    pos += w;
  }
  for (int t = 0; t < k.ntile; ++t) {
    idx[k.G + 1 + 2 * t] = vu[t * k.S];
    idx[k.G + 1 + 2 * t + 1] = vu[t * k.S + k.S - 1];
  }
  for (int v = 0; v < k.G; ++v)
    if (idx[v] < idx[v + 1]) k.J = std::max(k.J, (idx[v + 1] - 1) / k.S - idx[v] / k.S + 1);
  void* d = nullptr;
  TD3_RC(upload(h, owned, tiles.data(), tiles.size() * sizeof(DwTile), &d));
  k.tiles = static_cast<const DwTile*>(d);
  TD3_RC(upload(h, owned, idx.data(), idx.size() * sizeof(int), &d));
  k.wg_unit = static_cast<const int*>(d);
  k.tile_wg = k.wg_unit + k.G + 1;
  TD3_ARG(slab != nullptr, "internal: split-K dW stage without a plan slab");
  slab->bytes = std::max(slab->bytes, (size_t)k.G * k.J * k.slot * sizeof(float));
  out = k;
  return 0;
}

static int add_dw_stage(td3_handle* h, std::vector<void*>& owned, std::vector<Stage>& st,
                        Group& g, int which, const std::vector<BwdItem>& items, int Bp,
                        const char* tag, bool polyak, int enc_nwg = 0,
                        const std::vector<const float*>* unit_scale = nullptr, SlabRef* slab = nullptr) {
  const bool norm = h->cfg.norm == 1;
  const bool tile64 = Bp >= 512;
  std::vector<DwProb> probs;
  int blocks = 0;
  double flops = 0;
  double dw_operand_bytes = 0, dw_params = 0, dw_weights = 0;
  TD3_ARG(!unit_scale || unit_scale->size() == items.size(), "internal: one row scale per dW item");
  for (size_t k = 0; k < items.size(); ++k) {
    const BwdItem& it = items[k];
    const NetL& n = *it.net;
    const float* usc = unit_scale ? (*unit_scale)[k] : nullptr;
    for (int l = 0; l < 4; ++l) {
      const LinearL& L = n.lin[l];
      DwProb p{};
      p.rs = (usc && l < 3) ? usc : h->ones;
      p.ldrs = (usc && l < 3) ? 1 : 0;
      p.G = it.e->GZ[l];
      p.ldg = (l == 3) ? 32 : L.Np;
      p.U = (l == 0) ? (n.D > 0 ? it.e->Uin : it.e->X) : it.e->U[l - 1];
      p.ldu = (l == 0) ? ((n.D > 0 && norm) ? L.Kp : it.e->ldx) : n.lin[l - 1].Np;
      p.Np = L.Np;
      p.Kp = L.Kp;
      p.offW = L.offW;
      p.offb = L.offb;
      if (norm && l < 3) {
        p.offg = n.ln[l].offg;
        p.offbeta = n.ln[l].offb;
        p.GU = it.e->GU[l];
        p.ldgu = L.Np;
        p.H = it.e->H[l];
        p.ldh = L.Np;
        p.stats = it.e->stats[l];
      } else {
        p.offg = -1;
        p.offbeta = -1;
      }
      p.kvalid = L.K;
      p.ntk = tile64 ? (L.Kp + 63) / 64 : L.Kp / 32;
      p.tile_begin = blocks;
      blocks += (tile64 ? (L.Np + 63) / 64 : L.Np / 32) * p.ntk + L.Np / 32;
      flops += 2.0 * Bp * L.N * L.K;
      dw_operand_bytes += 4.0 * Bp * ((double)L.N + L.K) + ((norm && l < 3) ? 4.0 * Bp * (2.0 * L.N + 2.0) : 0.0);
      dw_params += (double)L.N * L.K + L.N + ((norm && l < 3) ? 2.0 * L.N : 0.0);
      dw_weights += (double)L.N * L.K;
      probs.push_back(p);
    }
    if (n.lnin) {
      DwProb p{};
      p.rs = usc ? usc : h->ones;
      p.ldrs = usc ? 1 : 0;
      p.Np = n.ln_in.Np;
      p.offb = -1;
      p.offg = n.ln_in.offg;
      p.offbeta = n.ln_in.offb;
      p.GU = it.e->GUin;
      p.ldgu = n.lin[0].Kp;
      p.H = it.e->X;
      p.ldh = it.e->ldx;
      p.stats = it.e->statsIn;
      p.ntk = 0;
      p.kvalid = 0;
      p.tile_begin = blocks;
      blocks += p.Np / 32;
      probs.push_back(p);
    }
  }
  TD3_ARG(probs.size() <= (size_t)kMaxDwProbs, "too many problems in one dw stage");
  DwArgs a{};
  for (size_t i = 0; i < probs.size(); ++i) a.probs[i] = probs[i];
  a.nprob = (int)probs.size();
  a.Bp = Bp;
  a.adam.P = g.P;
  a.adam.G = g.G;
  a.adam.M = g.M;
  a.adam.V = g.V;
  a.adam.T = g.T;
  a.adam.ctr = h->d_ctr;
  a.adam.which = which;
  a.adam.lr = h->adam[which].lr;
  a.adam.beta1 = h->adam[which].beta1;
  a.adam.beta2 = h->adam[which].beta2;
  a.adam.eps = h->adam[which].eps;
  a.adam.tau = (float)h->cfg.tau;
  a.adam.grad_scale = 1.0f;
  if (h->w4_build) {
    TD3_ARG(g.P4 && g.T4, "internal: k-quad images not allocated");
    a.adam.P4 = g.P4;
    a.adam.T4 = g.T4;
  }
  const bool dp = h->comm != nullptr || h->local != nullptr;
  const bool wn = g.wn.nlin > 0;
  a.mode = (dp || wn) ? kDwGrad : (polyak ? kDwAdamPolyak : kDwAdam);
  const double dw_bytes =
      dw_operand_bytes +
      (a.mode == kDwGrad ? 4.0 * dw_params
                         : dw_params * (a.mode == kDwAdamPolyak ? 32.0 : 24.0) +
                               (h->w4_build ? dw_weights * (a.mode == kDwAdamPolyak ? 8.0 : 4.0) : 0.0));
  a.tile64 = tile64 ? 1 : 0;
  a.scaled = unit_scale ? 1 : 0;
  const int tm = dwsk_tile_edge();
  const bool split = tile64 && Bp % 64 == 0 && TD3_DWSK;
  if (dp && split && !wn && enc_nwg == 0 && items.size() == 2 && dp_overlap(h)) {
    const bool local = h->local != nullptr;
    ncclComm_t comm = h->comm;
    hipStream_t cs = h->comm_stream;
    hipEvent_t ev = h->comm_ev, ev1 = h->comm_ev1, done = h->comm_done;
    TD3_ARG(local || (cs && ev && ev1 && done), "internal: data-parallel handle without a comm stream");
    const int pol = polyak ? 1 : 0;
    const std::string kname = std::string("td3::dwsk_kernel<") + (unit_scale ? "true, " : "false, ") +
                              (tm == 128 ? "true>" : "false>");
    int p0 = 0;
    std::vector<Stage> exch;
    for (size_t b = 0; b < items.size(); ++b) {
      const NetL& n = *items[b].net;
      const int cnt = 4 + (n.lnin ? 1 : 0);
      DwArgs ab = a;
      ab.nprob = cnt;
      double fb = 0;
      for (int i = 0; i < cnt; ++i) {
        ab.probs[i] = a.probs[p0 + i];
        if (i < 4) fb += 2.0 * Bp * n.lin[i].N * n.lin[i].K;
      }
      p0 += cnt;
      DwSplit kb{};
      TD3_RC(make_dw_split(h, owned, ab, slab, kb));
      const bool first = b == 0;
      const std::string bn = std::string(tag) + "_dw_" + std::to_string(b);
      st.push_back({bn,
                    [=](hipStream_t s) {
                      DwSplit kk = kb;
                      kk.slab = slab->p;
                      TD3_RC(launch_dw_split(ab, kk, s));
                      if (!local) TD3_HIP(hipEventRecord(first ? ev : ev1, s));
                      return 0;
                    },
                    fb, kname});
      const int64_t off = n.enc_off >= 0 ? n.enc_off : n.lin[0].offW;
      const int64_t end = b + 1 < items.size()
                              ? (items[b + 1].net->enc_off >= 0 ? items[b + 1].net->enc_off : items[b + 1].net->lin[0].offW)
                              : g.size;
      TD3_ARG(off >= 0 && end > off && end <= g.size, "internal: bucket range");
      const int64_t nb = end - off;
      AdamArgs ar = a.adam;
      ar.P += off; ar.G += off; ar.M += off; ar.V += off; ar.T += off;
      W4Map wm;
      TD3_RC(w4_map(h, g, off, &wm));
      ar.grad_scale = 1.0f / (float)h->nranks;
      float* Gb = g.G + off;
      Stage x{std::string(tag) + "_" + std::to_string(b) + "_allreduce",
              [=](hipStream_t s) {
                if (local) {
                  set_error("a td3_comm_init_local replica steps through td3_train_step_local only");
                  return -1;
                }
                TD3_HIP(hipStreamWaitEvent(cs, first ? ev : ev1, 0));
                ncclResult_t r = ncclAllReduce(Gb, Gb, (size_t)nb, ncclFloat, ncclSum, comm, cs);
                if (r != ncclSuccess) {
                  set_error("ncclAllReduce: %s", ncclGetErrorString(r));
                  return -2;
                }
                TD3_RC(launch_adam_flat(ar, nb, pol, cs, &wm));
                if (!first) TD3_HIP(hipEventRecord(done, cs));
                return 0;
              },
              0, "rccl"};
      x.collective = which == 1 ? 0 : 1;
      x.coll_off = off;
      x.coll_n = nb;
      x.after = [=](hipStream_t s) { return launch_adam_flat(ar, nb, pol, s, &wm); };
      exch.push_back(x);
    }
    for (auto& x : exch) st.push_back(x);
    st.push_back({std::string(tag) + "_join",
                  [=](hipStream_t s) {
                    if (local) return 0;
                    TD3_HIP(hipStreamWaitEvent(s, done, 0));
                    return 0;
                  },
                  0, "(stream join)"});
    return 0;
  }
  if (split) {
    DwSplit k{};
    TD3_RC(make_dw_split(h, owned, a, slab, k));
    st.push_back({std::string(tag) + "_dw",
                  [=](hipStream_t s) {
                    DwSplit kk = k;
                    kk.slab = slab->p;
                    return launch_dw_split(a, kk, s);
                  },
                  flops,
                  std::string("td3::dwsk_kernel<") + (unit_scale ? "true, " : "false, ") +
                      (tm == 128 ? "true>" : "false>")});
    st.back().bytes = dw_bytes;
  } else {
    st.push_back({std::string(tag) + "_dw", [=](hipStream_t s) { return launch_dw(a, blocks, s); }, flops,
                  std::string(tile64 ? "td3::dw64_kernel<" : "td3::dw_kernel<") + (unit_scale ? "true>" : "false>")});
    st.back().bytes = dw_bytes;
  }
  if (enc_nwg > 0) {
    EncAdamArgs ea{};
    for (auto& it : items) {
      if (it.net->D <= 0) continue;
      TD3_ARG(ea.nprob < 3, "too many encoders in one dw stage");
      ea.p[ea.nprob].partial = it.e->partial;
      ea.p[ea.nprob].off = it.net->enc_off;
      ea.nprob++;
    }
    ea.nwg = enc_nwg;
    ea.size = EncOff::size(items[0].net->D);
    ea.adam = a.adam;
    ea.mode = a.mode;
    st.push_back({std::string(tag) + "_enc_adam", [=](hipStream_t s) { return launch_enc_adam(ea, s); }, 0,
                  "td3::enc_adam_kernel"});
  }
  AdamArgs aa = a.adam;
  if (dp) aa.grad_scale = 1.0f / (float)h->nranks;
  const int pol = polyak ? 1 : 0;
  if (dp && !wn && dp_shard(h)) {
    const int N = h->nranks, R = h->rank;
    const int64_t slice = shard_slice(g, N);
    TD3_ARG(N * slice <= g.cap, "internal: shard slices past the arena");
    h->dp_sharded = true;
    ncclComm_t comm = h->comm;
    float* G = g.G;
    float* Pp = g.P;
    const bool local = h->local != nullptr;
    AdamArgs as = aa;
    as.P += R * slice; as.G += R * slice; as.M += R * slice; as.V += R * slice; as.T += R * slice;
    Stage x{std::string(tag) + "_rs_adam_ag",
            [=](hipStream_t s) {
              if (local) {
                set_error("a td3_comm_init_local replica steps through td3_train_step_local only");
                return -1;
              }
              ncclResult_t r = ncclReduceScatter(G, G + R * slice, (size_t)slice, ncclFloat, ncclSum, comm, s);
              if (r != ncclSuccess) {
                set_error("ncclReduceScatter: %s", ncclGetErrorString(r));
                return -2;
              }
              TD3_RC(launch_adam_flat(as, slice, 0, s));
              r = ncclAllGather(Pp + R * slice, Pp, (size_t)slice, ncclFloat, comm, s);
              if (r != ncclSuccess) {
                set_error("ncclAllGather: %s", ncclGetErrorString(r));
                return -2;
              }
              return 0;
            },
            0, "rccl"};
    x.collective = which == 1 ? 0 : 1;
    x.coll_slice = slice;
    x.after = [=](hipStream_t s) { return launch_adam_flat(as, slice, 0, s); };
    st.push_back(x);
    if (polyak && h->w4_build) {
      float* Tp = g.T;
      const int64_t n = g.size;
      const float tau = (float)h->cfg.tau;
      W4Map wm;
      TD3_RC(w4_map(h, g, 0, &wm));
      st.push_back({std::string(tag) + "_polyak", [=](hipStream_t s) { return launch_polyak_w4(Tp, Pp, n, tau, wm, s); },
                    0, "td3::polyak_w4_kernel"});
      return 0;
    }
    if (polyak) {
      float* Tp = g.T;
// ... 198 lines not shown
  const float* Pta = h->actor.T;
  const float* Pq1 = h->critic.P;
  const float* Pq2 = h->critic.P;
  const float* Ptq1 = h->critic.T;
  const float* Ptq2 = h->critic.T;

  const float ma = h->cfg.max_action;
  auto policy_head = [&](const float* Pp, EvalB& e, float* out, int target, int gen_noise) {
    return policy_head_prob(h, *P, Pp, e, {out, nullptr, P->ld_sa, sd, 1, ma}, target, gen_noise);
  };

  for (int actor_phase = 0; actor_phase < 2; ++actor_phase) {
    for (int inj = 0; inj < 2; ++inj) {
      std::vector<Stage>& st = P->body[actor_phase][inj];
      std::vector<FwdItem> f1 = {{&an, Pta, &P->TA, false, false}, {&q1, Pq1, &P->Q[0], true, true},
                                 {&q2, Pq2, &P->Q[1], true, true}};
      if (actor_phase) f1.push_back({&an, Pa, &P->A, true, true});
      TD3_RC(add_fwd_stages(h, P->tables, st, f1, Bp, B, "F", h->d_ctr, actor_phase, nullptr, nullptr, 0, true,
                            true));
      {
        std::vector<FwdItem> f1r = f1;
        f1r[0].ring_src = sd + ad;
        f1r[1].ring_src = 0;
        f1r[2].ring_src = 0;
        if (actor_phase) f1r[3].ring_src = 0;
        std::vector<Stage> fr;
        RingOut ro[4] = {{P->X_S2A, P->ld_sa, nullptr, 0, nullptr, nullptr},
                         {P->X_SA, P->ld_sa, nullptr, 0, nullptr, nullptr},
                         {nullptr, 0, nullptr, 0, P->R, P->ND},
                         {P->X_SP, P->ld_sa, nullptr, 0, nullptr, nullptr}};
        TD3_RC(add_fwd_stages(h, P->tables, fr, f1r, Bp, B, "F", h->d_ctr, actor_phase, &P->rside, ro,
                              2 * sd + ad, true, true));
        P->body_ring[actor_phase][inj].push_back(fr[0]);
      }
      {
        std::vector<GemmProb> hp = {policy_head(Pta, P->TA, P->X_S2A, 1, inj ? 0 : 1)};
        if (actor_phase) hp.push_back(policy_head(Pa, P->A, P->X_SP, 0, 0));
        const int n1 = (int)hp.size();
        for (int j = 0; j < 2; ++j) {
          const NetL& qj = j ? q2 : q1;
          GemmProb p{};
          p.norm = norm ? 1 : 0;
          p.B = B;
          set_ln3_head(p, Pq1, qj, P->Q[j]);
          p.ex[unit_loss::kQ] = P->Q[j].Qv;
          p.ex[unit_loss::kU3] = P->Q[j].U[2];
          p.ex[unit_loss::kStats3] = P->Q[j].stats[2];
          p.ex[unit_loss::kDU3] = P->Q[j].GU[2];
          p.Aout = P->Q[j].GZ[2];
          p.ldao = qj.lin[2].Np;
          hp.push_back(p);
        }
        TD3_RC(push_row2_stage(st, hp, kRowPolicyHead, kRowUnitLoss, n1, Bp, "heads"));
      }
      std::vector<BwdItem> cb = {{&q1, Pq1, &P->Q[0], true}, {&q2, Pq2, &P->Q[1], true}};
      std::vector<GemmProb> rows;
      {
        GemmProb p{};
        p.norm = norm ? 1 : 0;
        p.B = B;
        namespace tl = target_loss;
        for (int j = 0; j < 2; ++j) {
          const NetL& qj = j ? q2 : q1;
          const float* Ptq = j ? Ptq2 : Ptq1;
          p.ex[tl::kH3 + j] = P->TQ[j].H[2];
          p.ex[tl::kGamma3 + j] = const_cast<float*>(Ptq + qj.ln[2].offg);
          p.ex[tl::kBeta3 + j] = const_cast<float*>(Ptq + qj.ln[2].offb);
          p.ex[tl::kW4 + j] = const_cast<float*>(Ptq + qj.lin[3].offW);
          p.ex[tl::kB4 + j] = const_cast<float*>(Ptq + qj.lin[3].offb);
          p.ex[tl::kQ + j] = P->Q[j].Qv;
          p.ex[tl::kDZ4 + j] = P->Q[j].GZ[3];
          p.ex[tl::kG + j] = P->gscale[j];
        }
        p.ex[tl::kReward] = P->R;
        p.ex[tl::kNotDone] = P->ND;
        p.ex[tl::kY] = P->Y;
        p.ex[tl::kSqErr] = P->sqerr;
        p.exi[tl::kK3] = q1.lin[2].N;
        p.exi[tl::kLd3] = q1.lin[2].Np;
        p.exf[tl::kDiscount] = (float)h->cfg.discount;
        p.exf[tl::kGradScale] = (float)(2.0 / (double)B);
        rows.push_back(p);
      }
      TD3_RC(add_bwd_stages(h, P->tables, st, cb, Bp, B, "CB", true, false, &rows));
      std::vector<FwdItem> f2 = {{&q1, Ptq1, &P->TQ[0], false, false}, {&q2, Ptq2, &P->TQ[1], false, false}};
      TD3_RC(add_fwd_stages(h, P->tables, st, f2, Bp, B, "TF", nullptr, 0, nullptr, nullptr, 0, true));
      {
        const char* cbn[2] = {"CB_bwd2", "CB_bwd1"};
        std::vector<std::string> tfn;
        for (const char* n : {"TF_fwd0", "TF_fwd01", "TF_fwd1", "TF_fwd2"})
          if (stage_index(st, n) >= 0) tfn.push_back(n);
        for (size_t k = 0; k < 2 && k < tfn.size(); ++k) {
          const int i = stage_index(st, cbn[k]), j = stage_index(st, tfn[k]);
          if (i < 0 || j <= i || !merge_gemm_pair(st, (size_t)i, (size_t)j)) break;
        }
      }
      TD3_RC(push_row2_stage(st, rows, kRowTargetLoss, kRowLnBwd, 1, Bp, "critic_loss"));
      const std::vector<const float*> usc = {P->gscale[0], P->gscale[1]};
      TD3_RC(add_dw_stage(h, P->tables, st, h->critic, 0, cb, Bp, "C", actor_phase != 0, 0, &usc, &P->dwslab));
      if (!actor_phase) continue;
      std::vector<FwdItem> f3 = {{&q1, Pq1, &P->AQ, false, true}};
      const bool w1at = !can_fuse_l0(f3);
      if (w1at) {
        f3[0].tcopy = P->W1aT;
        f3[0].tcol = sd;
        f3[0].tn = ad;
      }
      TD3_RC(add_fwd_stages(h, P->tables, st, f3, Bp, B, "AF", nullptr, 0, nullptr, nullptr, 0, true, true));
      std::vector<BwdItem> aqb = {{&q1, Pq1, &P->AQ, false}};
      TD3_RC(add_bwd_stages(h, P->tables, st, aqb, Bp, B, "AQB", false, false, nullptr, (float)(-1.0) / (float)B));
      {
        GemmProb p{};
        p.norm = norm ? 1 : 0;
        p.B = B;
        namespace ab = actor_head_bwd;
        p.ex[ab::kDU0] = P->AQ.GU[0];
        p.ex[ab::kH0] = P->AQ.H[0];
        p.ex[ab::kStats0] = P->AQ.stats[0];
        p.ex[ab::kGamma0] = const_cast<float*>(Pq1 + q1.ln[0].offg);
        p.ex[ab::kW1] = const_cast<float*>(Pq1 + q1.lin[0].offW);
        p.ex[ab::kW1T] = w1at ? P->W1aT : nullptr;
        p.exi[ab::kLdW1T] = q1.lin[0].Np;
        p.exi[ab::kK0] = q1.lin[0].N;
        p.exi[ab::kLd0] = q1.lin[0].Np;
        p.exi[ab::kLdw1] = q1.lin[0].Kp;
        set_actor_bwd(p, Pa, an, P->A, sd, ad, ma);
        std::vector<GemmProb> v = {p};
        TD3_RC(push_row_stage(h, P->tables, st, v, kRowActorHeadBwd, Bp, "actor_head_bwd"));
      }
      std::vector<BwdItem> ab = {{&an, Pa, &P->A, true}};
      TD3_RC(add_bwd_stages(h, P->tables, st, ab, Bp, B, "AB", true));
      TD3_RC(add_dw_stage(h, P->tables, st, h->actor, 1, ab, Bp, "A", true, 0, nullptr, &P->dwslab));
    }
  }
  for (int a = 0; a < 2; ++a)
    for (int i = 0; i < 2; ++i) {
      std::vector<Stage>& br = P->body_ring[a][i];
      br.insert(br.end(), P->body[a][i].begin() + 1, P->body[a][i].end());
    }
  TD3_RC(alloc_dw_slab(P.get()));
  P->dp_overlap = (h->comm || h->local) && dp_overlap(h);
  if (h->plan) destroy_plan(h->plan.get());
  h->plan = std::move(P);
  return 0;
}

struct EncItem {
  const NetL* net;
  const float* P;
  float* X; int ldx;
  int next;
  uint64_t* mask;
};

static void push_enc_fwd(td3_handle* h, Plan* P, std::vector<Stage>& st, const std::vector<EncItem>& items,
                         const std::string& name) {
  const int N = h->N, D = h->D;
  const double flops = 2.0 * P->B * N * ((double)kEncC1 * D + (double)kEncC2 * kEncC1) * items.size();
  st.push_back({name,
                [=](hipStream_t s) {
                  EncFwdArgs a{};
                  for (size_t k = 0; k < items.size(); ++k) {
                    const EncItem& it = items[k];
                    a.p[k] = EncFwdProb{it.P + it.net->enc_off, it.next ? P->src_op2 : P->src_op, it.X, it.ldx,
                                        it.mask};
                  }
                  a.nprob = (int)items.size();
                  a.data = P->src_data;
                  a.rec = P->src_rec;
                  a.idx = P->src_idx;
                  a.B = P->B;
                  a.Bp = P->Bp;
                  a.N = N;
                  a.D = D;
                  a.ntile = (N + 31) / 32;
                  return launch_enc_fwd(a, s);
                },
                flops, "td3::enc_fwd_kernel<" + std::to_string(((D + 3) / 4) * 4) + ">"});
}

static int enc_bwd_nwg(int B, int nnets) { return std::max(1, std::min(B, 256 / std::max(1, nnets))); }

static void push_enc_bwd(td3_handle* h, Plan* P, std::vector<Stage>& st, const std::vector<BwdItem>& items,
                         const std::vector<float*>& X, const std::string& name) {
  const int N = h->N, D = h->D;
  const bool norm = h->cfg.norm == 1;
  const double flops = 2.0 * P->B * N * (2.0 * kEncC2 * kEncC1 + (double)kEncC1 * D) * items.size();
  st.push_back({name,
                [=](hipStream_t s) {
                  EncBwdArgs a{};
                  for (size_t k = 0; k < items.size(); ++k) {
                    const BwdItem& it = items[k];
                    EncBwdProb& q = a.p[k];
                    q.enc = it.P + it.net->enc_off;
                    q.part_off = P->src_op;
                    q.mask = it.e->mask;
                    q.X = X[k];
                    q.ldx = it.net->lin[0].Kp;
                    q.GU = it.e->GUin;
                    q.ldgu = it.net->lin[0].Kp;
                    q.stats = norm ? it.e->statsIn : nullptr;
                    q.gamma = it.P + it.net->ln_in.offg;
                    q.Kin = it.net->lin[0].K;
                    q.partial = it.e->partial;
                    q.gpool = it.e->gpool;
                  }
                  a.nprob = (int)items.size();
                  a.data = P->src_data;
                  a.rec = P->src_rec;
                  a.idx = P->src_idx;
                  a.B = P->B;
                  a.Bp = P->Bp;
                  a.N = N;
                  a.D = D;
                  a.ntile = (N + 31) / 32;
// ... 947 lines not shown
    off = 0;
    h->critic.nets.push_back(layout_mlp(h->sd + h->ad, cfg->critic_hidden, 1, norm, "q1.", off, h->critic.tensors));
    h->critic.nets.push_back(layout_mlp(h->sd + h->ad, cfg->critic_hidden, 1, norm, "q2.", off, h->critic.tensors));
    h->critic.size = off;
  }
  h->actor.cap = ((h->actor.size + 255) & ~(int64_t)255) + 256;
  h->critic.cap = ((h->critic.size + 255) & ~(int64_t)255) + 256;
  const size_t total = 7 * (size_t)(h->actor.cap + h->critic.cap);
  hipError_t e = hipMalloc(&h->arena, total * sizeof(float));
  if (e != hipSuccess) {
    set_error("td3_create: hipMalloc failed: %s", hipGetErrorString(e));
    delete h;
    return -2;
  }
  TD3_HIP(hipMemset(h->arena, 0, total * sizeof(float)));
  float* p = h->arena;
  for (Group* g : {&h->actor, &h->critic}) {
    g->P = p; p += g->cap;
    g->T = p; p += g->cap;
    g->M = p; p += g->cap;
    g->V = p; p += g->cap;
    g->G = p; p += g->cap;
    g->P4 = p; p += g->cap;
    g->T4 = p; p += g->cap;
  }
  TD3_HIP(hipMalloc(&h->d_ctr, sizeof(Counters)));
  {
    float one[64];
    for (float& v : one) v = 1.0f;
    TD3_HIP(hipMalloc(&h->ones, sizeof(one)));
    TD3_HIP(hipMemcpy(h->ones, one, sizeof(one), hipMemcpyHostToDevice));
  }
  {
    const Counters c0 = make_counters(h, 0, 0, 0);
    TD3_HIP(hipMemcpy(h->d_ctr, &c0, sizeof(c0), hipMemcpyHostToDevice));
  }
  if (norm == 2) {
    for (Group* g : {&h->actor, &h->critic}) {
      WnArgs& w = g->wn;
      for (const NetL& n : g->nets)
        for (const LinearL& L : n.lin) {
          TD3_ARG(w.nlin < kMaxWnLinears, "too many weight-normalised Linears");
          w.lin[w.nlin++] = WnLinear{L.offW, L.offb, L.offg, L.offv, L.N, L.K, L.Kp, w.rows};
          w.rows += L.N;
        }
    }
  }
  TD3_HIP(hipDeviceSynchronize());
  TD3_HIP(hipStreamCreateWithFlags(&h->stream, hipStreamNonBlocking));
  TD3_HIP(hipStreamCreateWithFlags(&h->act_stream, hipStreamNonBlocking));
  *out = h;
  return 0;
}

int td3_destroy(td3_handle* h) {
  if (!h) return 0;
  (void)hipSetDevice(h->cfg.device);
  (void)hipStreamSynchronize(h->stream);
  (void)hipStreamSynchronize(h->act_stream);
  ring_forget_stream(h->stream);
  if (h->plan) destroy_plan(h->plan.get());
  if (h->dev_stream && h->dev_stream != h->stream) (void)hipStreamSynchronize(h->dev_stream);
  if (h->dev_ev) (void)hipEventDestroy(h->dev_ev);
  for (auto* plans : {&h->act, &h->act_dev})
    for (auto& kv : *plans) {
      free_plan_tables(kv.second->tables);
      (void)hipFree(kv.second->scratch);
      if (kv.second->hio) (void)hipHostFree(kv.second->hio);
    }
  if (h->comm_stream) {
    (void)hipStreamSynchronize(h->comm_stream);
    (void)hipStreamDestroy(h->comm_stream);
    (void)hipEventDestroy(h->comm_ev);
    (void)hipEventDestroy(h->comm_ev1);
    (void)hipEventDestroy(h->comm_done);
  }
  if (h->comm) ncclCommDestroy(h->comm);
  if (h->local)
    for (auto& m : h->local->hs)
      if (m == h) m = nullptr;
  (void)hipFree(h->arena);
  (void)hipFree(h->d_ctr);
  (void)hipFree(h->ones);
  (void)hipStreamSynchronize(h->act_stream);
  (void)hipStreamDestroy(h->act_stream);
  if (h->actor_ev) (void)hipEventDestroy(h->actor_ev);
  (void)hipStreamDestroy(h->stream);
  delete h;
  return 0;
}

int td3_tensor_count(const td3_handle* h, int g) {
  if (!h) return -1;
  return (int)(g ? h->critic.tensors.size() : h->actor.tensors.size());
}

int td3_tensor_info(const td3_handle* h, int g, int i, char* name, int name_len, int64_t* rows,
                    int64_t* cols) {
  TD3_ARG(h != nullptr, "null handle");
  const Group& G = g ? h->critic : h->actor;
  TD3_ARG(i >= 0 && i < (int)G.tensors.size(), "tensor index out of range");
  const TensorRef& t = G.tensors[i];
  if (name && name_len > 0) snprintf(name, name_len, "%s", t.name.c_str());
  if (rows) *rows = t.rows;
  if (cols) *cols = t.cols;
  return 0;
}

int64_t td3_num_params(const td3_handle* h, int g) {
  if (!h) return -1;
  const Group& G = g ? h->critic : h->actor;
  int64_t n = 0;
  for (auto& t : G.tensors) n += t.rows * (t.cols ? t.cols : 1);
  return n;
}

static int which_ptr(td3_handle* h, int which, Group** g, float** base) {
  switch (which) {
    case TD3_ACTOR: *g = &h->actor; *base = h->actor.P; return 0;
    case TD3_ACTOR_TARGET: *g = &h->actor; *base = h->actor.T; return 0;
    case TD3_CRITIC: *g = &h->critic; *base = h->critic.P; return 0;
    case TD3_CRITIC_TARGET: *g = &h->critic; *base = h->critic.T; return 0;
    case TD3_ACTOR_ADAM_M: *g = &h->actor; *base = h->actor.M; return 0;
    case TD3_ACTOR_ADAM_V: *g = &h->actor; *base = h->actor.V; return 0;
    case TD3_CRITIC_ADAM_M: *g = &h->critic; *base = h->critic.M; return 0;
    case TD3_CRITIC_ADAM_V: *g = &h->critic; *base = h->critic.V; return 0;
    case TD3_ACTOR_GRAD: *g = &h->actor; *base = h->actor.G; return 0;
    case TD3_CRITIC_GRAD: *g = &h->critic; *base = h->critic.G; return 0;
  }
  set_error("unknown tensor group %d", which);
  return -1;
}

static int consolidate_moments(td3_handle* h, int which) {
  if (!h->dp_sharded || h->nranks <= 1) return 0;
  const bool m = which == TD3_ACTOR_ADAM_M || which == TD3_CRITIC_ADAM_M;
  const bool v = which == TD3_ACTOR_ADAM_V || which == TD3_CRITIC_ADAM_V;
  if (!m && !v) return 0;
  const bool actor = which == TD3_ACTOR_ADAM_M || which == TD3_ACTOR_ADAM_V;
  if (h->local) {
    const int64_t sl = shard_slice(actor ? h->actor : h->critic, h->nranks);
    for (int k = 0; k < (int)h->local->hs.size(); ++k) {
      td3_handle* o = h->local->hs[k];
      if (o == h || !o) continue;
      const Group& src = actor ? o->actor : o->critic;
      const Group& dst = actor ? h->actor : h->critic;
      TD3_HIP(hipMemcpy((m ? dst.M : dst.V) + k * sl, (m ? src.M : src.V) + k * sl, (size_t)sl * 4,
                        hipMemcpyDeviceToDevice));
    }
    return 0;
  }
  TD3_ARG(h->opt_gathered_it == h->total_it,
          "sharded optimizer state: call td3_dp_gather_optimizer_state on every rank before reading the "
          "Adam moments (a collective)");
  return 0;
}

int td3_dp_gather_optimizer_state(td3_handle* h) {
  TD3_ARG(h != nullptr, "null handle");
  TD3_HIP(hipSetDevice(h->cfg.device));
  if (h->dp_sharded && h->comm && h->nranks > 1) {
    if (h->last_step_stream && h->last_step_stream != h->stream) TD3_HIP(hipStreamSynchronize(h->last_step_stream));
    for (Group* g : {&h->actor, &h->critic}) {
      const int64_t sl = shard_slice(*g, h->nranks);
      for (float* a : {g->M, g->V}) {
        ncclResult_t r = ncclAllGather(a + h->rank * sl, a, (size_t)sl, ncclFloat, h->comm, h->stream);
        if (r != ncclSuccess) {
          set_error("ncclAllGather: %s", ncclGetErrorString(r));
          return -2;
        }
      }
    }
    TD3_HIP(hipStreamSynchronize(h->stream));
  }
  h->opt_gathered_it = h->total_it;
  return 0;
}

int td3_get_params(td3_handle* h, int which, float* out, int64_t n) {
  TD3_ARG(h && out, "null argument");
  Group* g;
  float* base;
  TD3_RC(which_ptr(h, which, &g, &base));
  TD3_ARG(n == td3_num_params(h, g == &h->critic), "size mismatch");
  TD3_HIP(hipSetDevice(h->cfg.device));
  TD3_HIP(hipStreamSynchronize(h->stream));
  TD3_HIP(hipDeviceSynchronize());
  TD3_RC(consolidate_moments(h, which));
  std::vector<float> host(g->size);
  TD3_HIP(hipMemcpy(host.data(), base, g->size * 4, hipMemcpyDeviceToHost));
  int64_t o = 0;
  for (auto& t : g->tensors) {
    if (t.cols) {
      for (int64_t r = 0; r < t.rows; ++r)
        memcpy(out + o + r * t.cols, host.data() + t.off + r * t.ld, t.cols * 4);
      o += t.rows * t.cols;
    } else {
      memcpy(out + o, host.data() + t.off, t.rows * 4);
      o += t.rows;
    }
  }
  return 0;
}

int td3_set_params(td3_handle* h, int which, const float* in, int64_t n) {
  TD3_ARG(h && in, "null argument");
  TD3_ARG(which != TD3_ACTOR_GRAD && which != TD3_CRITIC_GRAD, "the gradient arenas are read only");
  Group* g;
  float* base;
  TD3_RC(which_ptr(h, which, &g, &base));
  TD3_ARG(n == td3_num_params(h, g == &h->critic), "size mismatch");
  TD3_HIP(hipSetDevice(h->cfg.device));
  TD3_HIP(hipStreamSynchronize(h->stream));
  TD3_HIP(hipDeviceSynchronize());
  std::vector<float> host(g->size, 0.f);
  int64_t o = 0;
  for (auto& t : g->tensors) {
    if (t.cols) {
      for (int64_t r = 0; r < t.rows; ++r)
        memcpy(host.data() + t.off + r * t.ld, in + o + r * t.cols, t.cols * 4);
      o += t.rows * t.cols;
    } else {
      memcpy(host.data() + t.off, in + o, t.rows * 4);
      o += t.rows;
    }
  }
  TD3_HIP(hipMemcpy(base, host.data(), g->size * 4, hipMemcpyHostToDevice));
  if (base == g->P || base == g->T) g->w4_valid = false;
  if (g->wn.nlin > 0 && (base == g->P || base == g->T)) {
    WnArgs w = g->wn;
    w.mode = kWnDerive;
    w.arena = base;
    w.arena2 = nullptr;
    TD3_RC(launch_wn(w, h->stream));
    TD3_HIP(hipStreamSynchronize(h->stream));
  }
  return 0;
}

int td3_get_counters(const td3_handle* h, int64_t* total_it, int64_t* critic_step, int64_t* actor_step) {
  TD3_ARG(h != nullptr, "null handle");
  if (total_it) *total_it = h->total_it;
  if (critic_step) *critic_step = h->critic_step;
  if (actor_step) *actor_step = h->actor_step;
  return 0;
}

int td3_set_counters(td3_handle* h, int64_t total_it, int64_t critic_step, int64_t actor_step) {
  TD3_ARG(h != nullptr, "null handle");
  TD3_ARG(total_it >= 0 && critic_step >= 0 && actor_step >= 0, "negative counter");
  TD3_HIP(hipSetDevice(h->cfg.device));
  TD3_HIP(hipStreamSynchronize(h->stream));
  const Counters c = make_counters(h, total_it, critic_step, actor_step);
  TD3_HIP(hipMemcpy(h->d_ctr, &c, sizeof(c), hipMemcpyHostToDevice));
  h->total_it = total_it;
  h->critic_step = critic_step;
  h->actor_step = actor_step;
  return 0;
}

int td3_set_adam(td3_handle* h, int group, double lr, double beta1, double beta2, double eps) {
  TD3_ARG(h != nullptr, "null handle");
  TD3_ARG(group == 0 || group == 1, "group must be 0 (actor) or 1 (critic)");
  TD3_ARG(lr >= 0 && eps >= 0 && beta1 >= 0 && beta1 < 1 && beta2 >= 0 && beta2 < 1,
          "Adam hyper-parameters out of range (torch adam.py: 0 <= lr, eps; 0 <= betas < 1)");
  TD3_HIP(hipSetDevice(h->cfg.device));
  TD3_HIP(hipStreamSynchronize(h->stream));
  td3_handle::AdamHp& hp = h->adam[group == 0 ? 1 : 0];
  if (hp.lr == lr && hp.beta1 == beta1 && hp.beta2 == beta2 && hp.eps == eps) return 0;
  hp = td3_handle::AdamHp{lr, beta1, beta2, eps};
  const Counters c = make_counters(h, h->total_it, h->critic_step, h->actor_step);
  TD3_HIP(hipMemcpy(h->d_ctr, &c, sizeof(c), hipMemcpyHostToDevice));
  if (h->plan) TD3_RC(build_plan(h, h->plan->B));
  return 0;
}

int td3_get_adam(const td3_handle* h, int group, double out[4]) {
  TD3_ARG(h && out, "null argument");
  TD3_ARG(group == 0 || group == 1, "group must be 0 (actor) or 1 (critic)");
  const td3_handle::AdamHp& hp = h->adam[group == 0 ? 1 : 0];
  out[0] = hp.lr;
  out[1] = hp.beta1;
  out[2] = hp.beta2;
  out[3] = hp.eps;
  return 0;
}

int td3_train_step(td3_handle* h, rb_handle* rbh, int batch, void* stream, const int64_t* inject_idx,
                   const float* inject_noise, td3_step_stats* stats) {
  TD3_ARG(h && rbh, "null handle");
  TD3_ARG(batch > 0, "batch must be positive");
  Ring* r = reinterpret_cast<Ring*>(rbh);
  TD3_ARG(r->sd == h->sd && r->ad == h->ad, "replay buffer dims do not match the learner");
  TD3_ARG(r->size > 0 || inject_idx, "train on an empty replay buffer");
  TD3_ARG(r->device == h->cfg.device, "replay buffer lives on another device");
  TD3_HIP(hipSetDevice(h->cfg.device));
  TD3_ARG(r->particles == h->particles, "replay buffer kind does not match the learner");
  TD3_ARG(!r->particles || (r->N == h->N && r->D == h->D), "particle shape does not match the learner");
  TD3_RC(ensure_plan(h, batch));
  Plan* P = h->plan.get();
  TD3_RC(bind_ring(h, r));
  hipStream_t s = stream ? (hipStream_t)stream : h->stream;
  TD3_RC(ring_begin_read(r, s));
  if (inject_idx) {
    for (int i = 0; i < batch; ++i)
      TD3_ARG(inject_idx[i] >= 0 && inject_idx[i] < r->cap, "injected index out of range");
    TD3_HIP(hipMemcpyAsync(P->d_inject_idx, inject_idx, (size_t)batch * 8, hipMemcpyHostToDevice, s));
  }
  if (inject_noise)
    TD3_HIP(hipMemcpyAsync(P->noise, inject_noise, (size_t)batch * h->ad * 4, hipMemcpyHostToDevice, s));
  const int actor_phase = ((h->total_it + 1) % h->cfg.policy_freq) == 0;
  if (inject_idx) {
    TD3_RC(input_from_ring(h, r, P, true, s));
    TD3_RC(run_body(h, actor_phase, inject_noise ? 1 : 0, s, nullptr));
  } else {
    TD3_RC(run_body(h, actor_phase, inject_noise ? 1 : 0, s, r));
  }
  TD3_RC(ring_end_read(r, s));
  if (inject_idx || inject_noise) TD3_HIP(hipStreamSynchronize(s));
  return finish_step(h, actor_phase, s, stats);
}

int td3_train_step_batch(td3_handle* h, const float* state, const float* action, const float* next_state,
                         const float* reward, const float* not_done, int batch, void* stream,
                         const float* inject_noise, td3_step_stats* stats) {
  TD3_ARG(h != nullptr, "null handle");
  TD3_ARG(state && action && next_state && reward && not_done, "null input");
  TD3_ARG(batch > 0, "batch must be positive");
  TD3_ARG(!h->particles, "td3_train_step_batch on a particle learner (use td3_train_step_batch_particles)");
  TD3_HIP(hipSetDevice(h->cfg.device));
  TD3_RC(ensure_plan(h, batch));
  Plan* P = h->plan.get();
  hipStream_t s = stream ? (hipStream_t)stream : h->stream;
  if (inject_noise)
    TD3_HIP(hipMemcpyAsync(P->noise, inject_noise, (size_t)batch * h->ad * 4, hipMemcpyHostToDevice, s));
  const int actor_phase = ((h->total_it + 1) % h->cfg.policy_freq) == 0;
  TD3_RC(input_from_batch(h, P, state, action, next_state, reward, not_done, s));
  TD3_RC(run_body(h, actor_phase, inject_noise ? 1 : 0, s, nullptr));
  if (inject_noise) TD3_HIP(hipStreamSynchronize(s));
  return finish_step(h, actor_phase, s, stats);
}

static int put_rows(const ActPlan* A, float* dev, float* host, int ld, int col, const float* src, int n, int cols,
                    hipStream_t s) {
  if (!host) return copy_rows_h2d(dev, ld, col, src, n, cols, s);
  for (int i = 0; i < n; ++i) memcpy(host + (size_t)i * ld + col, src + (size_t)i * cols, (size_t)cols * 4);
  (void)A;
  return 0;
}

static int get_rows(float* dst, int cols, const float* dev, const float* host, int ld, int n, hipStream_t s) {
  if (host) {
    for (int i = 0; i < n; ++i) memcpy(dst + (size_t)i * cols, host + (size_t)i * ld, (size_t)cols * 4);
    return 0;
  }
  TD3_HIP(hipMemcpy2DAsync(dst, (size_t)cols * 4, dev, (size_t)ld * 4, (size_t)cols * 4, n, hipMemcpyDeviceToHost, s));
  TD3_HIP(hipStreamSynchronize(s));
  return 0;
}

static int wait_flags(volatile unsigned* f, int nprob, unsigned seq, hipStream_t s, int* ctr) {
  const auto t0 = std::chrono::steady_clock::now();
  const char* err = nullptr;
  for (int k = 0; k < nprob && !err; ++k) {
    int spin = 0;
    unsigned v;
    while ((v = f[k]) != seq && v != (seq | kActFailed)) {
      __builtin_ia32_pause();
      if ((++spin & 1023) == 0 && std::chrono::steady_clock::now() - t0 > std::chrono::seconds(2)) {
        TD3_HIP(hipStreamSynchronize(s));
        v = f[k];
        if (v != seq && v != (seq | kActFailed)) err = "the query kernel's completion flag did not arrive";
        break;
      }
    }
    if (!err && v == (seq | kActFailed)) err = "a query-kernel workgroup timed out waiting for layer 1 (outputs invalid)";
  }
  if (err) {
    TD3_HIP(hipStreamSynchronize(s));
    TD3_HIP(hipMemsetAsync(ctr, 0, sizeof(int) * 2 * nprob, s));
    TD3_HIP(hipStreamSynchronize(s));
    set_error("select_action / eval_q: %s", err);
    return -1;
  }
  std::atomic_thread_fence(std::memory_order_acquire);
  return 0;
}

static int run_gemv(const ActPlan* A, bool q, int n, const float* x0, int c0, const float* x1, int c1,
                    hipStream_t s) {
  const GemvArgs(&gv)[3] = q ? A->gv_q : A->gv_act;
  const int nprob = q ? 2 : 1;
  if (A->act1) {
    ActArgs a = q ? A->a1_q : A->a1_act;
    a.g.l1.B = n;
    const int K0 = c0 + c1;
    for (int r = 0; r < n; ++r) {
      memcpy(a.g.xq + r * K0, x0 + (size_t)r * c0, (size_t)c0 * 4);
      if (c1) memcpy(a.g.xq + r * K0 + c0, x1 + (size_t)r * c1, (size_t)c1 * 4);
    }
    ActPlan* M = const_cast<ActPlan*>(A);
    unsigned& sq = M->seq[q ? 1 : 0];
    sq = (sq + 1) & ~kActFailed;
    if (sq == 0) sq = 1;
    a.seq = sq;
    if (M->fail_test > 0) {
      a.fail_test = 1;
      --M->fail_test;
    }
    TD3_RC(launch_act(a, nprob, s));
    return wait_flags(M->hflag[q ? 1 : 0], nprob, a.seq, s, a.ctr);
  }
  int l = 0;
// ... 426 lines not shown
  for (int k = 0; k < n; ++k) {
    td3_handle* h = hs[k];
    Ring* r = reinterpret_cast<Ring*>(rbs[k]);
    TD3_ARG(r->sd == h->sd && r->ad == h->ad && r->particles == h->particles, "replay buffer does not match");
    TD3_ARG(!r->particles || (r->N == h->N && r->D == h->D), "particle replay buffer shape does not match");
    TD3_ARG(r->size > 0 || inject_idx, "train on an empty replay buffer");
    TD3_ARG(r->device == h->cfg.device, "replay buffer lives on another device");
    if (h->stream != s) TD3_HIP(hipStreamSynchronize(h->stream));
    TD3_RC(ensure_plan(h, batch));
    TD3_RC(ensure_w4(h, s));
    TD3_RC(bind_ring(h, r));
    TD3_RC(ring_begin_read(r, s));
  }
  const int actor_phase = ((h0->total_it + 1) % h0->cfg.policy_freq) == 0;
  const int inj = inject_noise ? 1 : 0;
  std::vector<std::vector<Stage>*> lists(n);
  std::vector<size_t> pos(n, 0);
  for (int k = 0; k < n; ++k) {
    td3_handle* h = hs[k];
    Plan* P = h->plan.get();
    Ring* r = reinterpret_cast<Ring*>(rbs[k]);
    if (inject_idx) {
      for (int i = 0; i < batch; ++i)
        TD3_ARG(inject_idx[(size_t)k * batch + i] >= 0 && inject_idx[(size_t)k * batch + i] < r->cap,
                "injected index out of range");
      TD3_HIP(hipMemcpyAsync(P->d_inject_idx, inject_idx + (size_t)k * batch, (size_t)batch * 8,
                             hipMemcpyHostToDevice, s));
    }
    if (inject_noise)
      TD3_HIP(hipMemcpyAsync(P->noise, inject_noise + (size_t)k * batch * h->ad, (size_t)batch * h->ad * 4,
                             hipMemcpyHostToDevice, s));
    const bool fused = !inject_idx && P->fuse_gather;
    if (!fused) TD3_RC(input_from_ring(h, r, P, inject_idx != nullptr, s));
    lists[k] = fused ? &P->body_ring[actor_phase][inj] : &P->body[actor_phase][inj];
    h->last_body = lists[k];
  }
  for (;;) {
    int coll = -2;
    for (int k = 0; k < n; ++k) {
      std::vector<Stage>& st = *lists[k];
      while (pos[k] < st.size() && st[pos[k]].collective < 0) TD3_RC(st[pos[k]++].run(s));
      const int c = pos[k] < st.size() ? st[pos[k]].collective : -1;
      TD3_ARG(k == 0 || c == coll, "internal: replicas reached different collectives");
      coll = c;
    }
    if (coll < 0) break;
    LocalSumArgs a{};
    a.n = n;
    std::vector<const Stage*> cst(n);
    for (int k = 0; k < n; ++k) {
      Group& grp = coll == 0 ? hs[k]->actor : hs[k]->critic;
      cst[k] = &(*lists[k])[pos[k]];
      a.a[k] = grp.G + cst[k]->coll_off;
      a.size = cst[k]->coll_n < 0 ? grp.size : cst[k]->coll_n;
      TD3_ARG(cst[k]->coll_off == cst[0]->coll_off && cst[k]->coll_n == cst[0]->coll_n,
              "internal: replicas reached different all-reduce buckets");
      ++pos[k];
    }
    TD3_RC(launch_local_sum(a, s));
    for (int k = 0; k < n; ++k)
      if (cst[k]->after) TD3_RC(cst[k]->after(s));
    const int64_t sl = cst[0]->coll_slice;
    if (sl > 0) {
      for (int k = 0; k < n; ++k) {
        const Group& own = coll == 0 ? hs[k]->actor : hs[k]->critic;
        for (int j = 0; j < n; ++j) {
          if (j == k) continue;
          const Group& dst = coll == 0 ? hs[j]->actor : hs[j]->critic;
          TD3_HIP(hipMemcpyAsync(dst.P + k * sl, own.P + k * sl, (size_t)sl * 4, hipMemcpyDeviceToDevice, s));
        }
      }
    }
  }
  for (int k = 0; k < n; ++k) TD3_RC(ring_end_read(reinterpret_cast<Ring*>(rbs[k]), s));
  if (inject_idx || inject_noise) TD3_HIP(hipStreamSynchronize(s));
  for (int k = 0; k < n; ++k) TD3_RC(finish_step(hs[k], actor_phase, s, stats ? &stats[k] : nullptr));
  return 0;
}

int td3_sync(td3_handle* h) {
  TD3_ARG(h != nullptr, "null handle");
  TD3_HIP(hipSetDevice(h->cfg.device));
  TD3_HIP(hipStreamSynchronize(h->stream));
  return 0;
}

void* td3_stream(td3_handle* h) { return h ? (void*)h->stream : nullptr; }

int td3_profile_stages(td3_handle* h, rb_handle* rbh, int batch, int actor_phase, float* ms, int max_stages,
                       int* n_stages) {
  TD3_ARG(h && rbh && ms && n_stages, "null argument");
  Ring* r = reinterpret_cast<Ring*>(rbh);
  TD3_HIP(hipSetDevice(h->cfg.device));
  TD3_RC(ensure_plan(h, batch));
  Plan* P = h->plan.get();
  TD3_RC(bind_ring(h, r));
  const bool fused = P->fuse_gather;
  std::vector<Stage>& st = fused ? P->body_ring[actor_phase ? 1 : 0][0] : P->body[actor_phase ? 1 : 0][0];
  const int n = (int)st.size() + 1;
  TD3_ARG(max_stages >= n, "max_stages too small");
  std::vector<hipEvent_t> ev(n + 1);
  for (auto& e : ev) TD3_HIP(hipEventCreate(&e));
  hipStream_t s = h->stream;
  TD3_RC(ensure_w4(h, s));
  TD3_RC(ring_begin_read(r, s));
  TD3_HIP(hipEventRecord(ev[0], s));
  if (!fused) TD3_RC(input_from_ring(h, r, P, false, s));
  TD3_HIP(hipEventRecord(ev[1], s));
  for (int i = 0; i < (int)st.size(); ++i) {
    TD3_RC(st[i].run(s));
    TD3_HIP(hipEventRecord(ev[i + 2], s));
  }
  TD3_RC(ring_end_read(r, s));
  TD3_HIP(hipStreamSynchronize(s));
  h->stage_names.clear();
  h->stage_kernels.clear();
  h->stage_names.push_back("gather");
  h->stage_kernels.push_back(fused ? "(fused into F_fwd0)" : "td3::gather_kernel");
  for (int i = 0; i < n; ++i) {
    TD3_HIP(hipEventElapsedTime(&ms[i], ev[i], ev[i + 1]));
    if (i) {
      h->stage_names.push_back(st[i - 1].name);
      h->stage_kernels.push_back(st[i - 1].kernel);
    }
  }
  for (auto& e : ev) (void)hipEventDestroy(e);
  *n_stages = n;
  h->last_body = &st;
  h->last_ring = r;
  h->last_ring_gen = r->gen;
  h->total_it += 1;
  h->critic_step += 1;
  if (actor_phase) h->actor_step += 1;
  return 0;
}

const char* td3_stage_name(td3_handle* h, int i) {
  if (!h || i < 0 || i >= (int)h->stage_names.size()) return "";
  return h->stage_names[i].c_str();
}

const char* td3_stage_kernel(td3_handle* h, int i) {
  if (!h || i < 0 || i >= (int)h->stage_kernels.size()) return "";
  return h->stage_kernels[i].c_str();
}

double td3_stage_flops(td3_handle* h, int i) {
  if (!h || !h->last_body || i <= 0 || i > (int)h->last_body->size()) return 0.0;
  return (*h->last_body)[i - 1].flops;
}

double td3_stage_bytes(td3_handle* h, int i) {
  if (!h || !h->last_body || i <= 0 || i > (int)h->last_body->size()) return 0.0;
  return (*h->last_body)[i - 1].bytes;
}

int td3_probe_kernel(td3_handle* h, rb_handle* rb, int batch, const char* kernel, int steps, float* ms_total,
                     int* launches) {
  TD3_ARG(h && rb && kernel && ms_total && launches, "null argument");
  TD3_ARG(steps > 0, "steps must be positive");
  TD3_ARG(!h->local, "a td3_comm_init_local replica steps through td3_train_step_local only");
  TD3_HIP(hipSetDevice(h->cfg.device));
  h->probing = true;
  h->probe_kernel = kernel;
  h->probe_used = 0;
  int rc = 0;
  for (int i = 0; i < steps && rc == 0; ++i) rc = td3_train_step(h, rb, batch, nullptr, nullptr, nullptr, nullptr);
// ... 97 lines not shown
```

Before: 10800 grad-steps/s.

## Fuse critic loss and LayerNorm-backward row work into dW kernel via tagged granules

Folds the per-row critic target/loss computation and the first-layer LayerNorm backward reductions into the weight-gradient kernel. Producer blocks publish per-row values as tagged 64-bit granules with relaxed atomics, and consumer tiles spin until tags match, then apply the dz0 transform in place. This removes separate row-stage and backward-dZ launches for the critic and actor. In exchange it relies on inter-block spinning, which is only safe if producers are co-resident, so it adds a timeout failure flag in mapped host memory plus host-side checks and granule resets.

```diff
diff --git a/include/td3.h b/include/td3.h
--- a/include/td3.h
+++ b/include/td3.h
@@ -160,6 +160,7 @@
 int td3_debug_plan_flags(const td3_handle* h, int* flags);
 
 int td3_debug_act_fail(td3_handle* h, int n);
+int td3_debug_dw_fail(td3_handle* h, int on);
 
 const char* td3_last_error(void);
 
diff --git a/td3_amd/_lib.py b/td3_amd/_lib.py
--- a/td3_amd/_lib.py
+++ b/td3_amd/_lib.py
@@ -107,6 +107,7 @@
     "td3_debug_activation": (C.c_int, [_P, C.c_int, C.c_int, _P, C.c_int, C.c_int]),
     "td3_debug_plan_flags": (C.c_int, [_P, _P]),
     "td3_debug_act_fail": (C.c_int, [_P, C.c_int]),
+    "td3_debug_dw_fail": (C.c_int, [_P, C.c_int]),
     "td3_last_error": (C.c_char_p, []),
 }
 
diff --git a/td3_amd/csrc/common.h b/td3_amd/csrc/common.h
--- a/td3_amd/csrc/common.h
+++ b/td3_amd/csrc/common.h
@@ -107,7 +107,7 @@
   int64_t total_it;
   int64_t critic_step;
   int64_t actor_step;
-  int64_t pad;
+  int64_t dw_fail_test;
   double pw[4];
   double beta[4];
 };
diff --git a/td3_amd/csrc/kernels.h b/td3_amd/csrc/kernels.h
--- a/td3_amd/csrc/kernels.h
+++ b/td3_amd/csrc/kernels.h
@@ -461,6 +461,27 @@
   int scaled;
 };
 
+constexpr int kDwFuseCritic = 1, kDwFuseActor = 2;
+constexpr int kDwFuseMaxRows = 480;
+constexpr int kDwFuseSpins = 1 << 15;
+struct DwFuseLn {
+  const float* GU; const float* H; const float* stats; const float* lng;
+  int ld, K;
+  int sums;
+  int gam;
+};
+struct DwFuse {
+  unsigned long long* gran;
+  unsigned* fail;
+  int nprod;
+  int nln;
+  DwFuseLn ln[2];
+  signed char pg[kMaxDwProbs], pz[kMaxDwProbs];
+  GemmProb tl;
+};
+int launch_dw_fused(const DwArgs& a, const DwFuse& f, int fuse, int norm, int nblocks, hipStream_t s);
+int dw_fused_blocks_per_cu(int fuse, int norm, int* out);
+
 struct DwTile {
   int prob;
   int kind;
diff --git a/td3_amd/csrc/kernels.hip b/td3_amd/csrc/kernels.hip
--- a/td3_amd/csrc/kernels.hip
+++ b/td3_amd/csrc/kernels.hip
@@ -902,8 +902,18 @@
   rv_store(P.Aout + (size_t)c.row * P.ldao, P.ldao, c.lane, gu[0]);
 }
 
-template <bool NORM>
-__device__ __forceinline__ void row_target_loss(const GemmProb& P, const RowCtx& c) {
+typedef GAS unsigned long long gu64;
+__device__ __forceinline__ void gran_store(unsigned long long* g, unsigned tag, float v) {
+  __hip_atomic_store((gu64*)g, ((unsigned long long)tag << 32) | __float_as_uint(v), __ATOMIC_RELAXED,
+                     __HIP_MEMORY_SCOPE_AGENT);
+}
+__device__ __forceinline__ unsigned long long gran_load(const unsigned long long* g) {
+  return __hip_atomic_load((gu64*)g, __ATOMIC_RELAXED, __HIP_MEMORY_SCOPE_AGENT);
+}
+
+template <bool NORM, bool GRAN = false>
+__device__ __forceinline__ void row_target_loss(const GemmProb& P, const RowCtx& c, unsigned long long* gran = nullptr,
+                                                unsigned tag = 0) {
   using namespace target_loss;
   asm volatile("" ::"s"(P.ex[kH3]), "s"(P.ex[kH3 + 1]), "s"(P.ex[kGamma3]), "s"(P.ex[kGamma3 + 1]), "s"(P.ex[kBeta3]),
                "s"(P.ex[kBeta3 + 1]), "s"(P.ex[kW4]), "s"(P.ex[kW4 + 1]), "s"(P.ex[kB4]), "s"(P.ex[kB4 + 1]),
@@ -941,12 +951,19 @@
   const float g1 = live ? P.exf[kGradScale] * e1 : 0.f, g2 = live ? P.exf[kGradScale] * e2 : 0.f;
   if (c.lane == 0) {
     gst(P.ex[kY] + c.row, y);
-    gst(P.ex[kDZ4] + ((size_t)c.row * 32), g1);
-    gst(P.ex[kDZ4 + 1] + ((size_t)c.row * 32), g2);
+    if constexpr (!GRAN) {
+      gst(P.ex[kDZ4] + ((size_t)c.row * 32), g1);
+      gst(P.ex[kDZ4 + 1] + ((size_t)c.row * 32), g2);
+    }
     gst(P.ex[kSqErr] + c.row, live ? e1 * e1 : 0.f);
     gst(P.ex[kSqErr] + (c.Bp + c.row), live ? e2 * e2 : 0.f);
-    gst(P.ex[kG] + c.row, g1);
-    gst(P.ex[kG + 1] + c.row, g2);
+    if constexpr (GRAN) {
+      gran_store(gran + c.row, tag, g1);
+      gran_store(gran + (c.Bp + c.row), tag, g2);
+    } else {
+      gst(P.ex[kG] + c.row, g1);
+      gst(P.ex[kG + 1] + c.row, g2);
+    }
   }
 }
 
@@ -2117,6 +2134,139 @@
   }
 }
 
+enum : int { kStG = 0, kStNm, kStRs, kStM1, kStNm2, kStN };
+constexpr int kDwRedFloats = 4 * 32 * 33;
+struct DwFuseCtx {
+  unsigned tag;
+  bool force;
+  float* stg;
+};
+
+template <int N>
+__device__ __forceinline__ void gran_sweep(const DwFuse& f, const DwFuseCtx& c, const int (&o)[N], float (&v)[N]) {
+  for (int spins = 0;; ++spins) {
+    bool ok = true;
+#pragma unroll
+    for (int k = 0; k < N; ++k) {
+      const unsigned long long x = gran_load(f.gran + o[k]);
+      v[k] = __uint_as_float((unsigned)x);
+      ok &= (unsigned)(x >> 32) == c.tag;
+    }
+    if (__all(ok) && !c.force) return;
+    if (c.force || spins >= kDwFuseSpins) {
+      if ((threadIdx.x & 63) == 0)
+        __hip_atomic_store((GAS unsigned*)f.fail, 0x80000000u | c.tag, __ATOMIC_RELAXED, __HIP_MEMORY_SCOPE_SYSTEM);
+      return;
+    }
+    __builtin_amdgcn_s_sleep(8);
+  }
+}
+
+template <int FUSE, bool NORM>
+__device__ __forceinline__ void dw_fuse_row(const DwFuse& f, int row, int e, bool first, int Bp, unsigned tag) {
+  constexpr int NL = FUSE == kDwFuseCritic ? 2 : 1;
+  const int lane = threadIdx.x & 63;
+  if constexpr (FUSE == kDwFuseCritic) row_target_loss<NORM, true>(f.tl, RowCtx{row, lane, Bp}, f.gran, tag);
+  if constexpr (NORM) {
+    float4 qg[NL][2], qu[NL][2], qh[NL][2];
+    float mean[NL], rstd[NL], gcp[NL];
+#pragma unroll
+    for (int k = 0; k < NL; ++k) {
+      const DwFuseLn& L = f.ln[k];
+      gcp[k] = gld(L.lng + min(e, L.ld - 1));
+      rv_load_raw(qg[k], L.lng, L.ld, lane);
+      rv_load_raw(qu[k], L.GU + (size_t)row * L.ld, L.ld, lane);
+      rv_load_raw(qh[k], L.H + (size_t)row * L.ld, L.ld, lane);
+      mean[k] = gld(L.stats + row);
+      rstd[k] = gld(L.stats + (Bp + row));
+    }
+#pragma unroll
+    for (int k = 0; k < NL; ++k) {
+      const DwFuseLn& L = f.ln[k];
+      if (first && e < L.ld) gran_store(f.gran + (L.gam + e), tag, gcp[k]);
+      float gu[8], h[8], g[8];
+      rv_from_raw(g, qg[k], L.ld, lane);
+      rv_from_raw(gu, qu[k], L.ld, lane);
+      rv_from_raw(h, qh[k], L.ld, lane);
+      const f32x2 rs = splat2(rstd[k]), nm = splat2(-mean[k]);
+      f32x2 gx[4], xh[4];
+#pragma unroll
+      for (int q = 0; q < 4; ++q) {
+        gx[q] = pk2(gu, q) * pk2(g, q);
+        xh[q] = (pk2(h, q) + nm) * rs;
+      }
+      const f32x2 sa = (gx[0] + gx[1]) + (gx[2] + gx[3]);
+      f32x2 sb = gx[0] * xh[0];
+      sb = pkfma(gx[1], xh[1], sb);
+      sb = pkfma(gx[2], xh[2], sb);
+      sb = pkfma(gx[3], xh[3], sb);
+      const float S1 = wsum(sa.x + sa.y), S2 = wsum(sb.x + sb.y);
+      if (lane == 0) {
+        gran_store(f.gran + ((size_t)L.sums * Bp + row), tag, S1);
+        gran_store(f.gran + ((size_t)(L.sums + 1) * Bp + row), tag, S2);
+      }
+    }
+  }
+}
+template <int FUSE, bool NORM>
+__device__ __forceinline__ void dw_fuse_rows(const DwFuse& f, int pidx, int Bp, unsigned tag) {
+  const int e = pidx * 256 + (int)threadIdx.x;
+  bool first = true;
+  for (int row = pidx * 4 + (int)(threadIdx.x >> 6); row < Bp; row += 4 * f.nprod, first = false)
+    dw_fuse_row<FUSE, NORM>(f, row, e, first, Bp, tag);
+}
+
+template <bool NORM>
+__device__ __forceinline__ float dz0_elem(float gu, float h, float gam, float nm, float rs, float m1, float nm2) {
+  if constexpr (!NORM) return h > 0.f ? gu : 0.f;
+  const float gx = gu * gam;
+  const float xh = (h + nm) * rs;
+  const float t = rs * __fmaf_rn(xh, nm2, gx - m1);
+  return h > 0.f ? t : 0.f;
+}
+
+template <bool SC, bool NORM, bool Z0, int NR, int NC>
+__device__ __forceinline__ void dw_stage_rows(const DwFuse& f, const DwFuseCtx& c, int pi, int Bp, const int (&r)[NR],
+                                              const int (&rc)[NR], const float (&mu)[NR], const float (&rs)[NR],
+                                              const int (&col)[NC], float (&gam)[NC]) {
+  constexpr bool LN = NORM && Z0;
+  constexpr int N = (SC ? NR : 0) + (LN ? 2 * NR + NC : 0);
+  if constexpr (N > 0) {
+    const DwFuseLn& L = f.ln[Z0 ? f.pz[pi] : 0];
+    int o[N];
+    float v[N];
+#pragma unroll
+    for (int j = 0; j < NR; ++j) {
+      if constexpr (SC) o[j] = f.pg[pi] * Bp + rc[j];
+      if constexpr (LN) {
+        o[(SC ? NR : 0) + j] = L.sums * Bp + rc[j];
+        o[(SC ? NR : 0) + NR + j] = (L.sums + 1) * Bp + rc[j];
+      }
+    }
+    if constexpr (LN) {
+#pragma unroll
+      for (int k = 0; k < NC; ++k) o[(SC ? NR : 0) + 2 * NR + k] = L.gam + col[k];
+    }
+    gran_sweep<N>(f, c, o, v);
+    const float invK = LN ? 1.0f / (float)L.K : 0.f;
+#pragma unroll
+    for (int j = 0; j < NR; ++j) {
+      if (r[j] < 0) continue;
+      if constexpr (SC) c.stg[kStG * kDwFuseMaxRows + r[j]] = v[j];
+      if constexpr (LN) {
+        c.stg[kStNm * kDwFuseMaxRows + r[j]] = -mu[j];
+        c.stg[kStRs * kDwFuseMaxRows + r[j]] = rs[j];
+        c.stg[kStM1 * kDwFuseMaxRows + r[j]] = v[(SC ? NR : 0) + j] * invK;
+        c.stg[kStNm2 * kDwFuseMaxRows + r[j]] = -(v[(SC ? NR : 0) + NR + j] * invK);
+      }
+    }
+    if constexpr (LN) {
+#pragma unroll
+      for (int k = 0; k < NC; ++k) gam[k] = v[(SC ? NR : 0) + 2 * NR + k];
+    }
+  }
+}
+
 template <int NT, bool SC>
 __device__ __forceinline__ void dw_vector_tile_cols(const DwArgs& a, const DwProb& P, const AdamK& k, int j,
                                                float* red) {
@@ -2248,9 +2398,156 @@
   TL_MARK(3);
 }
 
+template <int NT, bool SC, int U, int FZ, bool NORM>
+__device__ __forceinline__ void dw_vector_tile_fused(const DwArgs& a, const DwProb& P, const AdamPw& pw, int j,
+                                               float* red, const DwFuse* f, const DwFuseCtx* fc, int pi) {
+  constexpr int RG = NT / 8;
+  const int n0 = j * 32;
+  const int c4 = (threadIdx.x & 7) * 4, rg = threadIdx.x >> 3;
+  const bool ln = P.offg >= 0;
+  const bool hasb = P.offb >= 0;
+  const int c = threadIdx.x & 31;
+  const int64_t idx[3] = {P.offb + n0 + c, P.offg + n0 + c, P.offbeta + n0 + c};
+  const bool ok[3] = {hasb, ln, ln};
+  AdamState<3> st;
+  float sb[4] = {0.f, 0.f, 0.f, 0.f}, sg[4] = {0.f, 0.f, 0.f, 0.f}, sbeta[4] = {0.f, 0.f, 0.f, 0.f};
+  constexpr bool Z0 = FZ == 2;
+  const float* gzp = (hasb && !Z0) ? P.G : P.GU;
+  const float* gup = (ln || Z0) ? P.GU : P.G;
+  const float* hp = (ln || Z0) ? P.H : P.G;
+  const float* stp = ln ? P.stats : gup;
+  const int ldz = (hasb && !Z0) ? P.ldg : P.ldgu, ldu = (ln || Z0) ? P.ldgu : P.ldg, ldh = (ln || Z0) ? P.ldh : P.ldg;
+  for (int r0 = rg; r0 < a.Bp; r0 += RG * U) {
+    float4 gz[U], gu[U], hh[U];
+    float mu[U], rs[U], sc[U];
+#pragma unroll
+    for (int u = 0; u < U; ++u) {
+      const int r = min(r0 + RG * u, a.Bp - 1);
+      if constexpr (Z0) gz[u] = make_float4(0.f, 0.f, 0.f, 0.f);
+      else gz[u] = gld4(gzp + ((size_t)r * ldz + n0 + c4));
+      gu[u] = gld4(gup + ((size_t)r * ldu + n0 + c4));
+      hh[u] = gld4(hp + ((size_t)r * ldh + n0 + c4));
+      mu[u] = gld(stp + r);
+      rs[u] = gld(stp + (a.Bp + r));
+      sc[u] = (SC && !FZ) ? gld(P.rs + (size_t)r * P.ldrs) : 1.f;
+    }
+    if (r0 == rg && threadIdx.x < 32) adam_state_load<3>(a, idx, ok, st);
+    __builtin_amdgcn_sched_barrier(0);
+    [[maybe_unused]] float gam[4] = {0.f, 0.f, 0.f, 0.f};
+    if constexpr (FZ != 0) {
+      const int lane = threadIdx.x & 63;
+      const int sr = 8 * (int)(threadIdx.x >> 6) + (lane & 7) + 32 * (lane >> 3) + (r0 - rg);
+      const int r1[1] = {((lane >> 3) < U && sr < a.Bp) ? sr : -1}, rc1[1] = {min(sr, a.Bp - 1)};
+      const float unused[1] = {0.f};
+      const int col[4] = {n0 + c4, n0 + c4 + 1, n0 + c4 + 2, n0 + c4 + 3};
+      dw_stage_rows<SC, NORM, Z0, 1, 4>(*f, *fc, pi, a.Bp, r1, rc1, unused, unused, col, gam);
+      if constexpr (SC) {
+#pragma unroll
+        for (int u = 0; u < U; ++u) sc[u] = fc->stg[kStG * kDwFuseMaxRows + min(r0 + RG * u, a.Bp - 1)];
+      }
+    }
+    if (!hasb) {
+#pragma unroll
+      for (int u = 0; u < U; ++u) gz[u] = make_float4(0.f, 0.f, 0.f, 0.f);
+    }
+#pragma unroll
+    for (int u = 0; u < U; ++u) {
+      if (r0 + RG * u >= a.Bp) continue;
+      float z[4] = {gz[u].x * sc[u], gz[u].y * sc[u], gz[u].z * sc[u], gz[u].w * sc[u]};
+      if constexpr (Z0) {
+        const int r = r0 + RG * u;
+        const float m1 = NORM ? fc->stg[kStM1 * kDwFuseMaxRows + r] : 0.f;
+        const float nm2 = NORM ? fc->stg[kStNm2 * kDwFuseMaxRows + r] : 0.f;
+        const float u4[4] = {gu[u].x, gu[u].y, gu[u].z, gu[u].w}, h4[4] = {hh[u].x, hh[u].y, hh[u].z, hh[u].w};
+#pragma unroll
+        for (int e = 0; e < 4; ++e) z[e] = dz0_elem<NORM>(u4[e], h4[e], gam[e], -mu[u], rs[u], m1, nm2) * sc[u];
+      }
+      sb[0] += z[0]; sb[1] += z[1]; sb[2] += z[2]; sb[3] += z[3];
+      if (ln) {
+        const float g4[4] = {gu[u].x * sc[u], gu[u].y * sc[u], gu[u].z * sc[u], gu[u].w * sc[u]};
+        const float h4[4] = {hh[u].x, hh[u].y, hh[u].z, hh[u].w};
+#pragma unroll
+        for (int e = 0; e < 4; ++e) {
+          sg[e] += g4[e] * ((h4[e] - mu[u]) * rs[u]);
+          sbeta[e] += g4[e];
+        }
+      }
+    }
+  }
+#pragma unroll
+  for (int e = 0; e < 4; ++e) {
+    red[(0 * RG + rg) * 33 + c4 + e] = sb[e];
+    red[(1 * RG + rg) * 33 + c4 + e] = sg[e];
+    red[(2 * RG + rg) * 33 + c4 + e] = sbeta[e];
+  }
+  __syncthreads();
+  TL_MARK(1);
+  TL_MARK(2);
+  if (threadIdx.x < 32) {
+    float s0 = 0.f, s1 = 0.f, s2 = 0.f;
+#pragma unroll 8
+    for (int g = 0; g < RG; ++g) {
+      s0 += red[(0 * RG + g) * 33 + c];
+      s1 += red[(1 * RG + g) * 33 + c];
+      s2 += red[(2 * RG + g) * 33 + c];
+    }
+    const float gq[3] = {s0, s1, s2};
+    apply_grads_loaded<3>(a, make_adam(a.adam, pw), idx, gq, ok, st);
+  }
+  TL_MARK(3);
+}
+
 #ifndef TD3_DW_OCC
 #define TD3_DW_OCC 3
 #endif
+__device__ __forceinline__ void dw_matrix_finish(const DwArgs& a, const DwProb& P, const AdamPw& pw, const f32x16& acc,
+                                                 int n0, int k0, int64_t ix, float4 sm4, float4 sv4, float4 sp4,
+                                                 float4 st4, float* red) {
+  const int wave = threadIdx.x >> 6, lane = threadIdx.x & 63, i = lane & 31;
+  const int tn = threadIdx.x >> 3, tq = (threadIdx.x & 7) * 4;
+  const bool grad_only = a.mode == kDwGrad, pol = a.mode == kDwAdamPolyak;
+  TL_MARK(5);
+#pragma unroll
+  for (int r = 0; r < 16; ++r) red[(wave * 32 + mfma_row(r, lane)) * 33 + i] = acc[r];
+  __syncthreads();
+  TL_MARK(1);
+  TL_MARK(2);
+  const AdamK k = make_adam(a.adam, pw);
+  float gq[4];
+#pragma unroll
+  for (int q = 0; q < 4; ++q) {
+    float g = red[tn * 33 + tq + q];
+#pragma unroll
+    for (int w = 1; w < 4; ++w) g = g + red[(w * 32 + tn) * 33 + tq + q];
+    gq[q] = k0 + tq + q < P.kvalid ? g : 0.f;
+  }
+  if (grad_only) {
+    gst4(a.adam.G + ix, make_float4(gq[0], gq[1], gq[2], gq[3]));
+  } else {
+    float mm[4] = {sm4.x, sm4.y, sm4.z, sm4.w}, vv[4] = {sv4.x, sv4.y, sv4.z, sv4.w};
+    float pp[4] = {sp4.x, sp4.y, sp4.z, sp4.w}, tt[4] = {st4.x, st4.y, st4.z, st4.w};
+#pragma unroll
+    for (int e = 0; e < 4; ++e) {
+      mm[e] = __fmaf_rn(k.w1, gq[e] - mm[e], mm[e]);
+      vv[e] = vv[e] * k.b2;
+      vv[e] = vv[e] + (k.c2 * gq[e]) * gq[e];
+      const float denom = sqrtf(vv[e]) / k.bc2s + k.eps;
+      pp[e] = pp[e] + (k.negss * mm[e]) / denom;
+      tt[e] = k.tau * pp[e] + k.omt * tt[e];
+    }
+    sst4(a.adam.M + ix, make_float4(mm[0], mm[1], mm[2], mm[3]));
+    sst4(a.adam.V + ix, make_float4(vv[0], vv[1], vv[2], vv[3]));
+    pst4(a.adam.P + ix, make_float4(pp[0], pp[1], pp[2], pp[3]));
+    if (pol) pst4(a.adam.T + ix, make_float4(tt[0], tt[1], tt[2], tt[3]));
+    if (a.adam.P4) {
+      const int64_t iq = P.offW + ((int64_t)((k0 + tq) >> 2) * P.Np + n0 + tn) * 4;
+      pst4(a.adam.P4 + iq, make_float4(pp[0], pp[1], pp[2], pp[3]));
+      if (pol) pst4(a.adam.T4 + iq, make_float4(tt[0], tt[1], tt[2], tt[3]));
+    }
+  }
+  TL_MARK(3);
+}
+
 template <bool SC>
 __global__ __launch_bounds__(256, TD3_DW_OCC) void dw_kernel(DwArgs a, int nb) {
   __shared__ float red[4 * 32 * 33];
@@ -2343,6 +2640,139 @@
     return;
   }
   dw_vector_tile<256, SC>(a, P, pw, t - nmat, red);
+}
+
+template <bool Z0>
+__device__ __forceinline__ void dw_load_chunk_fused(const DwProb& P, int rc, int h, int n0, int k0, int i,
+                                                    float (&av)[16], float (&bv)[16], float (&hv)[Z0 ? 16 : 1]) {
+  const int rb = rc * 32 + 16 * h;
+  const int ldg = Z0 ? P.ldgu : P.ldg;
+  const float* gp = (Z0 ? P.GU : P.G) + (size_t)rb * ldg + n0 + i;
+  const float* up = P.U + (size_t)rb * P.ldu + k0 + i;
+#pragma unroll
+  for (int s = 0; s < 16; ++s) {
+    av[s] = gld(gp + (size_t)s * ldg);
+    bv[s] = gld(up + (size_t)s * P.ldu);
+  }
+  if constexpr (Z0) {
+    const float* hp = P.H + (size_t)rb * P.ldh + n0 + i;
+#pragma unroll
+    for (int s = 0; s < 16; ++s) hv[s] = gld(hp + (size_t)s * P.ldh);
+  }
+}
+template <bool SC, bool NORM, bool Z0>
+__device__ __forceinline__ void dw_xform_chunk(float (&av)[16], const float (&hv)[Z0 ? 16 : 1], const float* stg, int rb,
+                                               float gam) {
+#pragma unroll
+  for (int q = 0; q < 4; ++q) {
+    const float* p = stg + rb + 4 * q;
+    float4 g4 = make_float4(1.f, 1.f, 1.f, 1.f), nm4 = g4, rs4 = g4, m14 = g4, nm24 = g4;
+    if constexpr (SC) g4 = *reinterpret_cast<const float4*>(p + kStG * kDwFuseMaxRows);
+    if constexpr (Z0 && NORM) {
+      nm4 = *reinterpret_cast<const float4*>(p + kStNm * kDwFuseMaxRows);
+      rs4 = *reinterpret_cast<const float4*>(p + kStRs * kDwFuseMaxRows);
+      m14 = *reinterpret_cast<const float4*>(p + kStM1 * kDwFuseMaxRows);
+      nm24 = *reinterpret_cast<const float4*>(p + kStNm2 * kDwFuseMaxRows);
+    }
+    const float g[4] = {g4.x, g4.y, g4.z, g4.w}, nm[4] = {nm4.x, nm4.y, nm4.z, nm4.w}, rs[4] = {rs4.x, rs4.y, rs4.z, rs4.w};
+    const float m1[4] = {m14.x, m14.y, m14.z, m14.w}, nm2[4] = {nm24.x, nm24.y, nm24.z, nm24.w};
+#pragma unroll
+    for (int e = 0; e < 4; ++e) {
+      float v = av[4 * q + e];
+      if constexpr (Z0) v = dz0_elem<NORM>(v, hv[4 * q + e], gam, nm[e], rs[e], m1[e], nm2[e]);
+      if constexpr (SC) v *= g[e];
+      av[4 * q + e] = v;
+    }
+  }
+}
+template <bool SC, bool NORM, bool Z0>
+__device__ __forceinline__ void dw_matrix_tile_fused(const DwArgs& a, const DwProb& P, const DwFuse& f,
+                                                     const DwFuseCtx& c, int pi, int t, const AdamPw& pw, float* red) {
+  constexpr int NH = Z0 ? 16 : 1;
+  const int kt = t % P.ntk, nt = t / P.ntk;
+  const int n0 = nt * 32, k0 = kt * 32;
+  const int wave = threadIdx.x >> 6, lane = threadIdx.x & 63;
+  const int i = lane & 31, h = lane >> 5;
+  const int nrc = a.Bp >> 5;
+  const int cb = wave * nrc / 4, ce = (wave + 1) * nrc / 4;
+  f32x16 acc;
+#pragma unroll
+  for (int r = 0; r < 16; ++r) acc[r] = 0.f;
+  float a0[16], b0[16], a1[16], b1[16], h0[NH], h1[NH];
+  if (cb < ce) dw_load_chunk_fused<Z0>(P, cb, h, n0, k0, i, a0, b0, h0);
+  if (cb + 1 < ce) dw_load_chunk_fused<Z0>(P, cb + 1, h, n0, k0, i, a1, b1, h1);
+  const int tn = threadIdx.x >> 3, tq = (threadIdx.x & 7) * 4;
+  const int64_t ix = P.offW + (int64_t)(n0 + tn) * P.Kp + k0 + tq;
+  const bool pol = a.mode == kDwAdamPolyak;
+  float4 sm4 = make_float4(0.f, 0.f, 0.f, 0.f), sv4 = sm4, sp4 = sm4, st4 = sm4;
+  auto load_state = [&]() {
+    sm4 = gld4(a.adam.M + ix), sv4 = gld4(a.adam.V + ix), sp4 = gld4(a.adam.P + ix);
+    st4 = gld4((pol ? a.adam.T : a.adam.P) + ix);
+  };
+  if (!Z0 || cb >= ce) load_state();
+  float gam[1] = {0.f};
+  if (cb < ce) {
+    int r[2], rc[2];
+    float mu[2] = {0.f, 0.f}, rs[2] = {0.f, 0.f};
+#pragma unroll
+    for (int j = 0; j < 2; ++j) {
+      const int x = 32 * cb + lane + 64 * j;
+      r[j] = x < 32 * ce ? x : -1;
+      rc[j] = min(x, 32 * ce - 1);
+      if constexpr (Z0 && NORM) {
+        mu[j] = gld(P.stats + rc[j]);
+        rs[j] = gld(P.stats + (a.Bp + rc[j]));
+      }
+    }
+    const int col[1] = {n0 + i};
+    TL_MARK(6);
+    dw_stage_rows<SC, NORM, Z0, 2, 1>(f, c, pi, a.Bp, r, rc, mu, rs, col, gam);
+    TL_MARK(7);
+  }
+  for (int rc = cb; rc < ce; rc += 2) {
+    dw_xform_chunk<SC, NORM, Z0>(a0, h0, c.stg, rc * 32 + 16 * h, gam[0]);
+#pragma unroll
+    for (int s = 0; s < 16; ++s) acc = mfma32x32x2(a0[s], b0[s], acc);
+    if (Z0 && rc == cb) load_state();
+    if (rc + 2 < ce) dw_load_chunk_fused<Z0>(P, rc + 2, h, n0, k0, i, a0, b0, h0);
+    if (rc + 1 >= ce) break;
+    dw_xform_chunk<SC, NORM, Z0>(a1, h1, c.stg, (rc + 1) * 32 + 16 * h, gam[0]);
+#pragma unroll
+    for (int s = 0; s < 16; ++s) acc = mfma32x32x2(a1[s], b1[s], acc);
+    if (rc + 3 < ce) dw_load_chunk_fused<Z0>(P, rc + 3, h, n0, k0, i, a1, b1, h1);
+  }
+  dw_matrix_finish(a, P, pw, acc, n0, k0, ix, sm4, sv4, sp4, st4, red);
+}
+
+template <bool SC, int FUSE, bool NORM>
+__global__ __launch_bounds__(256, TD3_DW_OCC) void dw_kernel(DwArgs a, int nb, DwFuse f) {
+  __shared__ __attribute__((aligned(16))) float red[kDwRedFloats + kStN * kDwFuseMaxRows];
+  const int b = xcd_tile(nb);
+  TL_MARK(0);
+  if (b >= nb) return;
+  const Counters* ctr = a.adam.ctr;
+  const DwFuseCtx c{(unsigned)(a.adam.which ? ctr->actor_step : ctr->critic_step) + 1u, ctr->dw_fail_test != 0,
+                    red + kDwRedFloats};
+  if constexpr (FUSE == kDwFuseCritic || NORM) {
+    if (b < f.nprod) dw_fuse_rows<FUSE, NORM>(f, b, a.Bp, c.tag);
+  }
+  int pi = 0;
+#pragma unroll
+  for (int i = 1; i < kMaxDwProbs; ++i)
+    if (i < a.nprob && b >= a.probs[i].tile_begin) pi = i;
+  const DwProb& P = a.probs[pi];
+  const int t = b - P.tile_begin;
+  const int nmat = (P.Np >> 5) * P.ntk;
+  const AdamPw pw = adam_pw(a.adam);
+  const bool z0 = f.pz[pi] >= 0;
+  if (t < nmat) {
+    if (z0) dw_matrix_tile_fused<SC, NORM, true>(a, P, f, c, pi, t, pw, red);
+    else dw_matrix_tile_fused<SC, NORM, false>(a, P, f, c, pi, t, pw, red);
+    return;
+  }
+  if (z0) dw_vector_tile_fused<256, SC, 4, 2, NORM>(a, P, pw, t - nmat, red, &f, &c, pi);
+  else if constexpr (SC) dw_vector_tile_fused<256, SC, 4, 1, NORM>(a, P, pw, t - nmat, red, &f, &c, pi);
+  else dw_vector_tile<256, SC>(a, P, pw, t - nmat, red);
 }
 
 constexpr int kDw64S = 66;
@@ -3430,6 +3860,39 @@
   return 0;
 }
 
+template <typename F>
+static int dw_fused_select(int fuse, int norm, F&& fn) {
+  if (fuse == kDwFuseCritic) return norm ? fn(dw_kernel<true, kDwFuseCritic, true>) : fn(dw_kernel<true, kDwFuseCritic, false>);
+  if (fuse == kDwFuseActor) return norm ? fn(dw_kernel<false, kDwFuseActor, true>) : fn(dw_kernel<false, kDwFuseActor, false>);
+  set_error("internal: dW fuse kind %d", fuse);
+  return -1;
+}
+
+int launch_dw_fused(const DwArgs& a, const DwFuse& f, int fuse, int norm, int nblocks, hipStream_t s) {
+  if (nblocks <= 0 || a.tile64 || a.mode == kDwGrad || a.Bp > kDwFuseMaxRows || (a.scaled != 0) != (fuse == kDwFuseCritic) ||
+      !f.gran || !f.fail) {
+    set_error("launch_dw_fused: not a fused dW launch (%d tiles, Bp %d, mode %d)", nblocks, a.Bp, a.mode);
+    return -1;
+  }
+  const dim3 grid((nblocks + 7) & ~7);
+  TD3_RC(dw_fused_select(fuse, norm, [&](auto* k) {
+    hipLaunchKernelGGL(k, grid, dim3(256), 0, s, a, nblocks, f);
+    return 0;
+  }));
+  TD3_HIP(hipGetLastError());
+  return 0;
+}
+
+int dw_fused_blocks_per_cu(int fuse, int norm, int* out) {
+  int n = 0;
+  TD3_RC(dw_fused_select(fuse, norm, [&](auto* k) {
+    TD3_HIP(hipOccupancyMaxActiveBlocksPerMultiprocessor(&n, k, 256, 0));
+    return 0;
+  }));
+  *out = std::min(std::min(n, 8), 800 / (((102 + 6 + 15) / 16) * 16 + 16));
+  return 0;
+}
+
 int launch_dw_split(const DwArgs& a, const DwSplit& k, hipStream_t s) {
   if (k.ntile <= 0) return 0;
   if (k.G <= 0 || (k.G & 7) || k.S <= 0 || (a.Bp & 63) || a.Bp != 64 * k.S || (k.tm != 64 && k.tm != 128) ||
diff --git a/td3_amd/csrc/td3.hip b/td3_amd/csrc/td3.hip
--- a/td3_amd/csrc/td3.hip
+++ b/td3_amd/csrc/td3.hip
@@ -189,6 +189,8 @@
   int ld_sa = 0;
   float *R = nullptr, *ND = nullptr, *noise = nullptr, *Y = nullptr, *sqerr = nullptr;
   float* gscale[2] = {};
+  unsigned long long* gran[2] = {};
+  size_t gran_bytes[2] = {};
   float* W1aT = nullptr;
   int64_t* d_idx = nullptr;
   int64_t* d_inject_idx = nullptr;
@@ -286,6 +288,8 @@
   float* arena = nullptr;
   Counters* d_ctr = nullptr;
   float* ones = nullptr;
+  unsigned* dw_fail = nullptr;
+  unsigned* dw_fail_dev = nullptr;
   int64_t total_it = 0, critic_step = 0, actor_step = 0;
   struct AdamHp { double lr, beta1, beta2, eps; } adam[2];
   hipStream_t stream = nullptr;
@@ -999,10 +1003,36 @@
   return 0;
 }
 
+struct DwFuseReq {
+  int kind = 0;
+  GemmProb tl{};
+  unsigned long long** gran = nullptr;
+  size_t* gran_bytes = nullptr;
+};
+
+static int dw_fuse_ok(td3_handle* h, const std::vector<BwdItem>& items, int Bp, int kind, bool* ok) {
+  *ok = false;
+  if (env_int("TD3_FUSE_ROWS", 0) == 0) return 0;
+  if (h->particles || h->cfg.norm == 2 || h->comm || h->local || Bp >= 512 || Bp > kDwFuseMaxRows) return 0;
+  int blocks = 0;
+  for (auto& it : items) {
+    const NetL& n = *it.net;
+    if (n.lnin || n.D > 0 || n.lin[0].Np > 512) return 0;
+    for (int l = 0; l < 4; ++l) blocks += (n.lin[l].Np / 32) * (n.lin[l].Kp / 32) + n.lin[l].Np / 32;
+  }
+  int per_cu = 0, cus = 0;
+  TD3_RC(dw_fused_blocks_per_cu(kind, h->cfg.norm == 1, &per_cu));
+  TD3_HIP(hipDeviceGetAttribute(&cus, hipDeviceAttributeMultiprocessorCount, h->cfg.device));
+  if (blocks > cus * per_cu || blocks < 2) return 0;
+  *ok = true;
+  return 0;
+}
+
 static int add_dw_stage(td3_handle* h, std::vector<void*>& owned, std::vector<Stage>& st,
                         Group& g, int which, const std::vector<BwdItem>& items, int Bp,
                         const char* tag, bool polyak, int enc_nwg = 0,
-                        const std::vector<const float*>* unit_scale = nullptr, SlabRef* slab = nullptr) {
+                        const std::vector<const float*>* unit_scale = nullptr, SlabRef* slab = nullptr,
+                        const DwFuseReq* fuse = nullptr) {
   const bool norm = h->cfg.norm == 1;
   const bool tile64 = Bp >= 512;
   std::vector<DwProb> probs;
@@ -1038,6 +1068,15 @@
       } else {
         p.offg = -1;
         p.offbeta = -1;
+      }
+      if (fuse && l == 0) {
+        p.G = it.e->GU[0];
+        p.ldg = L.Np;
+        p.GU = it.e->GU[0];
+        p.ldgu = L.Np;
+        p.H = it.e->H[0];
+        p.ldh = L.Np;
+        p.stats = it.e->stats[0];
       }
       p.kvalid = L.K;
       p.ntk = tile64 ? (L.Kp + 63) / 64 : L.Kp / 32;
@@ -1184,7 +1223,72 @@
                   0, "(stream join)"});
     return 0;
   }
-  if (split) {
+  if (fuse) {
+    const bool critic = fuse->kind == kDwFuseCritic;
+    TD3_ARG(!tile64 && a.mode != kDwGrad && enc_nwg == 0 && items.size() <= 2 && a.nprob == 4 * (int)items.size() &&
+                (unit_scale != nullptr) == critic,
+            "internal: this dW stage cannot take its row launch");
+    DwFuse f{};
+    f.tl = fuse->tl;
+    f.nln = norm ? (int)items.size() : 0;
+    f.nprod = (critic || norm) ? std::min(Bp / 4, blocks) : 0;
+    int slots = critic ? 2 : 0;
+    double row_bytes = 0, row_flops = 0;
+    for (size_t k = 0; k < items.size(); ++k) {
+      const NetL& n = *items[k].net;
+      const LinearL& L0 = n.lin[0];
+      if (norm) {
+        DwFuseLn& L = f.ln[k];
+        L.GU = items[k].e->GU[0];
+        L.H = items[k].e->H[0];
+        L.stats = items[k].e->stats[0];
+        L.lng = items[k].P + n.ln[0].offg;
+        L.ld = L0.Np;
+        L.K = L0.N;
+        L.sums = slots;
+        slots += 2;
+      }
+      row_bytes += (norm ? 4.0 * Bp * (2.0 * L0.N + 2.0) : 4.0 * Bp * L0.N) + (critic ? 4.0 * Bp * (n.lin[2].N + 4.0) : 0.0);
+      row_flops += (norm ? 14.0 : 1.0) * Bp * L0.N + (critic ? 20.0 * Bp * n.lin[2].N : 0.0);
+      if (critic) {
+        std::vector<float> e((size_t)Bp * 32, 0.f);
+        for (int r = 0; r < Bp; ++r) e[(size_t)r * 32] = 1.f;
+        TD3_HIP(hipMemcpy(items[k].e->GZ[3], e.data(), e.size() * 4, hipMemcpyHostToDevice));
+      }
+    }
+    int ngran = slots * Bp;
+    for (int k = 0; k < f.nln; ++k) {
+      f.ln[k].gam = ngran;
+      ngran += f.ln[k].ld;
+    }
+    for (int i = 0; i < a.nprob; ++i) {
+      f.pg[i] = critic ? (signed char)(i / 4) : (signed char)-1;
+      f.pz[i] = i % 4 == 0 ? (signed char)(i / 4) : (signed char)-1;
+    }
+    TD3_ARG(fuse->gran && fuse->gran_bytes, "internal: fused dW stage without a granule block");
+    if (!*fuse->gran) {
+      *fuse->gran_bytes = ((size_t)std::max(ngran, 2) * 8 + 15) & ~(size_t)15;
+      void* d = nullptr;
+      TD3_HIP(hipMalloc(&d, *fuse->gran_bytes));
+      TD3_HIP(hipMemset(d, 0, *fuse->gran_bytes));
+      owned.push_back(d);
+      *fuse->gran = static_cast<unsigned long long*>(d);
+    }
+    if (!h->dw_fail) {
+      TD3_HIP(hipHostMalloc(&h->dw_fail, 64, hipHostMallocMapped));
+      memset(h->dw_fail, 0, 64);
+      void* d = nullptr;
+      TD3_HIP(hipHostGetDevicePointer(&d, h->dw_fail, 0));
+      h->dw_fail_dev = static_cast<unsigned*>(d);
+    }
+    f.gran = *fuse->gran;
+    f.fail = h->dw_fail_dev;
+    const int kind = fuse->kind, nrm = norm ? 1 : 0;
+    st.push_back({std::string(tag) + "_dw", [=](hipStream_t s) { return launch_dw_fused(a, f, kind, nrm, blocks, s); },
+                  flops + row_flops,
+                  std::string("td3::dw_kernel<") + (critic ? "true, 1, " : "false, 2, ") + (norm ? "true>" : "false>")});
+    st.back().bytes = dw_bytes + row_bytes;
+  } else if (split) {
     DwSplit k{};
     TD3_RC(make_dw_split(h, owned, a, slab, k));
     st.push_back({std::string(tag) + "_dw",
@@ -1549,7 +1653,9 @@
         p.exf[tl::kGradScale] = (float)(2.0 / (double)B);
         rows.push_back(p);
       }
-      TD3_RC(add_bwd_stages(h, P->tables, st, cb, Bp, B, "CB", true, false, &rows));
+      bool fuse_c = false;
+      TD3_RC(dw_fuse_ok(h, cb, Bp, kDwFuseCritic, &fuse_c));
+      TD3_RC(add_bwd_stages(h, P->tables, st, cb, Bp, B, "CB", !fuse_c, false, &rows));
       std::vector<FwdItem> f2 = {{&q1, Ptq1, &P->TQ[0], false, false}, {&q2, Ptq2, &P->TQ[1], false, false}};
       TD3_RC(add_fwd_stages(h, P->tables, st, f2, Bp, B, "TF", nullptr, 0, nullptr, nullptr, 0, true));
       {
@@ -1562,9 +1668,18 @@
           if (i < 0 || j <= i || !merge_gemm_pair(st, (size_t)i, (size_t)j)) break;
         }
       }
-      TD3_RC(push_row2_stage(st, rows, kRowTargetLoss, kRowLnBwd, 1, Bp, "critic_loss"));
       const std::vector<const float*> usc = {P->gscale[0], P->gscale[1]};
-      TD3_RC(add_dw_stage(h, P->tables, st, h->critic, 0, cb, Bp, "C", actor_phase != 0, 0, &usc, &P->dwslab));
+      if (fuse_c) {
+        DwFuseReq fr;
+        fr.kind = kDwFuseCritic;
+        fr.tl = rows[0];
+        fr.gran = &P->gran[0];
+        fr.gran_bytes = &P->gran_bytes[0];
+        TD3_RC(add_dw_stage(h, P->tables, st, h->critic, 0, cb, Bp, "C", actor_phase != 0, 0, &usc, &P->dwslab, &fr));
+      } else {
+        TD3_RC(push_row2_stage(st, rows, kRowTargetLoss, kRowLnBwd, 1, Bp, "critic_loss"));
+        TD3_RC(add_dw_stage(h, P->tables, st, h->critic, 0, cb, Bp, "C", actor_phase != 0, 0, &usc, &P->dwslab));
+      }
       if (!actor_phase) continue;
       std::vector<FwdItem> f3 = {{&q1, Pq1, &P->AQ, false, true}};
       const bool w1at = !can_fuse_l0(f3);
@@ -1596,8 +1711,18 @@
         TD3_RC(push_row_stage(h, P->tables, st, v, kRowActorHeadBwd, Bp, "actor_head_bwd"));
       }
       std::vector<BwdItem> ab = {{&an, Pa, &P->A, true}};
-      TD3_RC(add_bwd_stages(h, P->tables, st, ab, Bp, B, "AB", true));
-      TD3_RC(add_dw_stage(h, P->tables, st, h->actor, 1, ab, Bp, "A", true, 0, nullptr, &P->dwslab));
+      bool fuse_a = false;
+      TD3_RC(dw_fuse_ok(h, ab, Bp, kDwFuseActor, &fuse_a));
+      TD3_RC(add_bwd_stages(h, P->tables, st, ab, Bp, B, "AB", !fuse_a));
+      if (fuse_a) {
+        DwFuseReq fr;
+        fr.kind = kDwFuseActor;
+        fr.gran = &P->gran[1];
+        fr.gran_bytes = &P->gran_bytes[1];
+        TD3_RC(add_dw_stage(h, P->tables, st, h->actor, 1, ab, Bp, "A", true, 0, nullptr, &P->dwslab, &fr));
+      } else {
+        TD3_RC(add_dw_stage(h, P->tables, st, h->actor, 1, ab, Bp, "A", true, 0, nullptr, &P->dwslab));
+      }
     }
   }
   for (int a = 0; a < 2; ++a)
@@ -2711,6 +2836,7 @@
   (void)hipFree(h->arena);
   (void)hipFree(h->d_ctr);
   (void)hipFree(h->ones);
+  if (h->dw_fail) (void)hipHostFree(h->dw_fail);
   (void)hipStreamSynchronize(h->act_stream);
   (void)hipStreamDestroy(h->act_stream);
   if (h->actor_ev) (void)hipEventDestroy(h->actor_ev);
@@ -2875,11 +3001,43 @@
   return 0;
 }
 
+static int zero_dw_granules(td3_handle* h) {
+  if (!h->plan) return 0;
+  for (int k = 0; k < 2; ++k)
+    if (h->plan->gran[k]) TD3_HIP(hipMemsetAsync(h->plan->gran[k], 0, h->plan->gran_bytes[k], h->stream));
+  TD3_HIP(hipStreamSynchronize(h->stream));
+  return 0;
+}
+
+static int check_dw_fail(td3_handle* h) {
+  if (!h->dw_fail || !*(volatile unsigned*)h->dw_fail) return 0;
+  TD3_HIP(hipStreamSynchronize(h->stream));
+  if (h->last_step_stream && h->last_step_stream != h->stream) TD3_HIP(hipStreamSynchronize(h->last_step_stream));
+  const unsigned word = *(volatile unsigned*)h->dw_fail;
+  *(volatile unsigned*)h->dw_fail = 0;
+  const int64_t off = 0;
+  TD3_HIP(hipMemcpy(&h->d_ctr->dw_fail_test, &off, sizeof(off), hipMemcpyHostToDevice));
+  TD3_RC(zero_dw_granules(h));
+  set_error("a fused dW launch gave up waiting for its row granules (step tag %u): the results of that step are invalid",
+            word & 0x7fffffffu);
+  return -3;
+}
+
+int td3_debug_dw_fail(td3_handle* h, int on) {
+  TD3_ARG(h != nullptr, "null handle");
+  TD3_HIP(hipSetDevice(h->cfg.device));
+  TD3_HIP(hipStreamSynchronize(h->stream));
+  const int64_t v = on ? 1 : 0;
+  TD3_HIP(hipMemcpy(&h->d_ctr->dw_fail_test, &v, sizeof(v), hipMemcpyHostToDevice));
+  return 0;
+}
+
 int td3_set_counters(td3_handle* h, int64_t total_it, int64_t critic_step, int64_t actor_step) {
   TD3_ARG(h != nullptr, "null handle");
   TD3_ARG(total_it >= 0 && critic_step >= 0 && actor_step >= 0, "negative counter");
   TD3_HIP(hipSetDevice(h->cfg.device));
   TD3_HIP(hipStreamSynchronize(h->stream));
+  TD3_RC(zero_dw_granules(h));
   const Counters c = make_counters(h, total_it, critic_step, actor_step);
   TD3_HIP(hipMemcpy(h->d_ctr, &c, sizeof(c), hipMemcpyHostToDevice));
   h->total_it = total_it;
@@ -2926,6 +3084,7 @@
   TD3_HIP(hipSetDevice(h->cfg.device));
   TD3_ARG(r->particles == h->particles, "replay buffer kind does not match the learner");
   TD3_ARG(!r->particles || (r->N == h->N && r->D == h->D), "particle shape does not match the learner");
+  TD3_RC(check_dw_fail(h));
   TD3_RC(ensure_plan(h, batch));
   Plan* P = h->plan.get();
   TD3_RC(bind_ring(h, r));
@@ -2958,6 +3117,7 @@
   TD3_ARG(batch > 0, "batch must be positive");
   TD3_ARG(!h->particles, "td3_train_step_batch on a particle learner (use td3_train_step_batch_particles)");
   TD3_HIP(hipSetDevice(h->cfg.device));
+  TD3_RC(check_dw_fail(h));
   TD3_RC(ensure_plan(h, batch));
   Plan* P = h->plan.get();
   hipStream_t s = stream ? (hipStream_t)stream : h->stream;
@@ -3550,7 +3710,7 @@
   TD3_ARG(h != nullptr, "null handle");
   TD3_HIP(hipSetDevice(h->cfg.device));
   TD3_HIP(hipStreamSynchronize(h->stream));
-  return 0;
+  return check_dw_fail(h);
 }
 
 void* td3_stream(td3_handle* h) { return h ? (void*)h->stream : nullptr; }
```

Result: no change. 10770 grad-steps/s (-0.4%).
